# facebookresearch/fast3r

Measured on AMD Instinct MI355X. Metric: views/sec (512^2, ViT-L) single forward pass at N=320, higher is better.
Workload: dtype fp16

## Files before the change

fast3r_amd/_lib.py:

```python
import ctypes
import os

import torch

F3R_F16, F3R_BF16 = 0, 1
F3R_A_PLAIN, F3R_A_CONV3X3 = 0, 1
F3R_EPI_GENERIC, F3R_EPI_QKV, F3R_EPI_CONVT = 0, 1, 2
F3R_ACT_NONE, F3R_ACT_GELU, F3R_ACT_RELU = 0, 1, 2
F3R_SPLIT_NONE, F3R_SPLIT_W2, F3R_SPLIT_X3, F3R_SPLIT_W2F8, F3R_SPLIT_X3F8 = 0, 1, 2, 3, 4
F3R_MAX_SEG = 8
F3R_REAL_F32, F3R_REAL_F64 = 0, 1
F3R_LOSS_DIS, F3R_LOSS_LOG1P = 0, 1
SCENE_TILE = 4096
COLLECT_TILE = 1024
F3R_SKY_CLASSIFY, F3R_SKY_MORPH, F3R_SKY_LABEL = 1, 2, 4
F3R_SKY_EMPTY, F3R_SKY_NO_TOP, F3R_SKY_TOP = 0, 1, 2
SKY_PIX_TILE, SKY_WORD_TILE = 16, 256
MESH_TILE = 1024
F3R_INDEX_I32, F3R_INDEX_I64 = 0, 1
CLOUD_TILE, CLOUD_SORT_TILE, CLOUD_FPS_TILE, CLOUD_FPS_ONE_MAX = 1024, 2048, 1024, 8192
RENDER_CENTER_PARTS = 1024
RASTER_SMALL_PIXELS = 64
F3R_FPS_AUTO, F3R_FPS_ONE, F3R_FPS_TILED = 0, 1, 2
MAPS_TILE = 1024
F3R_MAPS_LUT, F3R_MAPS_RGB = 0, 1
GTVIEW_CAM_WORDS = 25
F3R_GTVIEW_POSE, F3R_GTVIEW_FINITE_MASK = 1, 2
DEPTH_TILE, DEPTH_ROW_WORDS, DEPTH_OUT_WORDS, DEPTH_MAX_THRESHOLDS = 1024, 8, 16, 4
F3R_DEPTH_ALIGN_NONE, F3R_DEPTH_ALIGN_MEDIAN = 0, 1
MATCH_TILE = 2048
F3R_CLEAN_WORLD, F3R_CLEAN_CAMERA = 0, 1
F3R_GALIGN_L1, F3R_GALIGN_L2 = 0, 1

_c_i64, _c_i32, _c_f32, _c_vp = ctypes.c_int64, ctypes.c_int32, ctypes.c_float, ctypes.c_void_p


class GemmArgs(ctypes.Structure):
    _fields_ = [
        ("A", _c_vp), ("W", _c_vp), ("bias", _c_vp),
        ("M", _c_i64), ("N", _c_i32), ("K", _c_i32), ("Kpad", _c_i32), ("lda", _c_i64),
        ("a_mode", _c_i32), ("a_relu", _c_i32),
        ("conv_H", _c_i32), ("conv_W", _c_i32), ("conv_C", _c_i32), ("conv_stride", _c_i32),
        ("conv_OH", _c_i32), ("conv_OW", _c_i32),
        ("epi", _c_i32), ("act", _c_i32),
        ("rowadd", _c_vp), ("rowadd_div", _c_i64),
        ("res_f32", _c_vp), ("ldr_f32", _c_i64),
        ("res_lp", _c_vp), ("ldr_lp", _c_i64),
        ("res_lp2", _c_vp), ("ldr_lp2", _c_i64),
        ("out_f32", _c_vp), ("ldo_f32", _c_i64),
        ("out_lp", _c_vp), ("ldo_lp", _c_i64),
        ("q", _c_vp), ("k", _c_vp), ("vt", _c_vp), ("seq_len", _c_i64), ("ldvt", _c_i64),
        ("rope_cos", _c_vp), ("rope_sin", _c_vp), ("rope_w", _c_i32), ("q_scale", _c_f32),
        ("ct_s", _c_i32), ("ct_h", _c_i32), ("ct_w", _c_i32), ("ct_cout", _c_i32),
        ("dtype", _c_i32), ("rope_mode", _c_i32),
        ("split", _c_i32), ("kernel_sel", _c_i32), ("A_lo", _c_vp),
        ("out_lp_lo", _c_vp), ("res_lp_lo", _c_vp), ("res_lp2_lo", _c_vp), ("out_relu", _c_vp), ("out_relu_lo", _c_vp),
        ("qkv_dq", _c_i32), ("out_lp_f8", _c_i32),
        ("w_scale", _c_vp), ("W_aux", _c_vp),
        ("out_f8", _c_vp), ("out_relu_f8", _c_vp),
        ("fin_w", _c_vp), ("fin_b", _c_vp), ("fin_pts", _c_vp), ("fin_conf", _c_vp),
        ("fin_n_out", _c_i32), ("fin_depth_mode", _c_i32), ("fin_conf_mode", _c_i32), ("fin_vmin", _c_f32), ("fin_vmax", _c_f32), ("reserved0", _c_i32),
    ]


class AttnArgs(ctypes.Structure):
    _fields_ = [
        ("q", _c_vp), ("o", _c_vp),
        ("ldq", _c_i64), ("ldo", _c_i64),
        ("q_batch_stride", _c_i64), ("o_batch_stride", _c_i64),
        ("tq", _c_i64),
        ("batch", _c_i32), ("n_heads", _c_i32), ("n_seg", _c_i32), ("dtype", _c_i32),
        ("k_seg", _c_vp * F3R_MAX_SEG), ("vt_seg", _c_vp * F3R_MAX_SEG),
        ("seg_len", _c_i64 * F3R_MAX_SEG), ("ldvt", _c_i64 * F3R_MAX_SEG),
        ("ldk", _c_i64),
        ("k_batch_stride", _c_i64 * F3R_MAX_SEG), ("vt_batch_stride", _c_i64 * F3R_MAX_SEG),
        ("scale", _c_f32), ("q_prescaled", _c_i32),
        ("st_o", _c_vp), ("st_ml", _c_vp), ("state_in", _c_i32), ("state_out", _c_i32),
        ("kv_group", _c_i32), ("causal", _c_i32), ("q_pos0", _c_i64), ("seg_pos0", _c_i64 * F3R_MAX_SEG),
        ("kernel_sel", _c_i32), ("head_dim", _c_i32),
        ("dbg_counters", _c_vp),
        ("sched_counter", _c_vp),
        ("qk_planes", _c_i32), ("reserve_cus", _c_i32),
    ]


class AttnF32Args(ctypes.Structure):
    _fields_ = [
        ("q", _c_vp), ("k", _c_vp), ("v", _c_vp), ("ldq", _c_i64), ("ldkv", _c_i64),
        ("o_hi", _c_vp), ("o_lo", _c_vp), ("o_f32", _c_vp), ("ldo", _c_i64),
        ("n_seq", _c_i64), ("tq", _c_i64), ("tk", _c_i64), ("q_pos0", _c_i64), ("k_pos0", _c_i64),
        ("n_heads", _c_i32), ("kv_group", _c_i32), ("causal", _c_i32), ("dtype", _c_i32), ("head_dim", _c_i32), ("scale", _c_f32),
    ]


SYMBOLS = {
    "f3r_version": (ctypes.c_int, []),
    "f3r_last_error_string": (ctypes.c_char_p, []),
    "f3r_sizeof": (ctypes.c_size_t, [ctypes.c_int]),
    "f3r_wall_clock_khz": (ctypes.c_int, []),
    "f3r_patchify": (ctypes.c_int, [_c_vp, _c_vp, ctypes.c_int, ctypes.c_int, ctypes.c_int, ctypes.c_int, ctypes.c_int, ctypes.c_int, _c_vp]),
    "f3r_interp_bilinear": (ctypes.c_int, [_c_vp, _c_vp, _c_vp, _c_vp] + [ctypes.c_int] * 9 + [_c_vp]),
    "f3r_interp_bilinear_f8": (ctypes.c_int, [_c_vp, _c_vp, _c_vp, _c_vp, _c_vp] + [ctypes.c_int] * 9 + [_c_vp]),
    "f3r_layernorm": (ctypes.c_int, [_c_vp, _c_vp, _c_vp, _c_vp, _c_vp, _c_i64, ctypes.c_int, _c_f32, ctypes.c_int, ctypes.c_int, _c_vp]),
    "f3r_layernorm_f8": (ctypes.c_int, [_c_vp, _c_vp, _c_vp, _c_vp, _c_i64, _c_i64, ctypes.c_int, _c_f32, ctypes.c_int, _c_vp]),
    "f3r_gemm": (ctypes.c_int, [ctypes.POINTER(GemmArgs), _c_vp]),
    "f3r_attn_fwd": (ctypes.c_int, [ctypes.POINTER(AttnArgs), _c_vp]),
    "f3r_attn_kernel_name": (ctypes.c_char_p, [ctypes.POINTER(AttnArgs)]),
    "f3r_block_workspace_bytes": (ctypes.c_size_t, [_c_i64, ctypes.c_int, ctypes.c_int, ctypes.c_int, _c_i64, _c_i64, ctypes.POINTER(ctypes.c_size_t)]),
    "f3r_block_workspace_bytes_ex": (ctypes.c_size_t, [_c_i64, ctypes.c_int, ctypes.c_int, ctypes.c_int, _c_i64, _c_i64, ctypes.c_int, ctypes.POINTER(ctypes.c_size_t)]),
    "f3r_upsample2x": (ctypes.c_int, [_c_vp, _c_vp, _c_vp, _c_vp, ctypes.c_int, ctypes.c_int, ctypes.c_int, ctypes.c_int, ctypes.c_int, ctypes.c_int, ctypes.c_int, _c_vp]),
    "f3r_dpt_final": (ctypes.c_int, [_c_vp, _c_vp, _c_vp, _c_vp, ctypes.c_int, _c_vp, _c_vp, _c_i64, ctypes.c_int, ctypes.c_int, ctypes.c_int,
                                     _c_f32, _c_f32, ctypes.c_int, _c_vp]),
    "f3r_cast_f32_to_lp": (ctypes.c_int, [_c_vp, _c_vp, _c_vp, _c_i64, ctypes.c_int, _c_vp]),
    "f3r_align_workspace_bytes": (ctypes.c_size_t, [ctypes.c_int]),
    "f3r_align_local_to_global": (ctypes.c_int, [_c_vp, _c_vp, _c_vp, _c_vp, _c_vp, _c_vp, _c_vp, _c_vp, ctypes.c_size_t,
                                                 ctypes.c_int, _c_i64, _c_f32, _c_vp]),
    "f3r_focal_workspace_bytes": (ctypes.c_size_t, [ctypes.c_int, ctypes.c_int, ctypes.c_int]),
    "f3r_estimate_focal": (ctypes.c_int, [_c_vp, _c_vp, _c_vp, _c_vp, _c_vp, ctypes.c_size_t, ctypes.c_int, ctypes.c_int, ctypes.c_int,
                                          _c_f32, _c_f32, _c_f32, ctypes.c_int, _c_f32, _c_f32, _c_vp]),
    "f3r_nn_index_bytes": (ctypes.c_size_t, [_c_i64]),
    "f3r_nn_workspace_bytes": (ctypes.c_size_t, [_c_i64]),
    "f3r_nn_build": (ctypes.c_int, [_c_vp, _c_i64, _c_vp, ctypes.c_size_t, _c_vp, ctypes.c_size_t, _c_vp]),
    "f3r_nn_query": (ctypes.c_int, [_c_vp, _c_vp, _c_i64, _c_vp, _c_vp, _c_vp, ctypes.c_size_t, _c_vp]),
    "f3r_estimate_normals": (ctypes.c_int, [_c_vp, _c_vp, ctypes.c_int, _c_vp, _c_vp, _c_vp, _c_vp]),
    "f3r_recon_stats_workspace_bytes": (ctypes.c_size_t, [_c_i64]),
    "f3r_recon_stats": (ctypes.c_int, [_c_vp, _c_vp, _c_vp, _c_vp, _c_i64, _c_i64, ctypes.c_double, _c_vp, _c_vp, ctypes.c_size_t, _c_vp]),
    "f3r_recon_prepare_workspace_bytes": (ctypes.c_size_t, [ctypes.c_int, ctypes.c_int, _c_i64]),
    "f3r_recon_prepare": (ctypes.c_int, [_c_vp, _c_vp, _c_vp, _c_vp, _c_vp, ctypes.c_int, ctypes.c_int, _c_i64, _c_f32, _c_f32, _c_vp, _c_vp,
                                         _c_vp, _c_vp, _c_vp, ctypes.c_size_t, _c_vp]),
    "f3r_resample_u8": (ctypes.c_int, [_c_vp, _c_vp, ctypes.c_int, ctypes.c_int, ctypes.c_int, ctypes.c_int, _c_vp, _c_vp, ctypes.c_int, _c_vp]),
    "f3r_imgnorm_u8": (ctypes.c_int, [_c_vp, _c_vp, ctypes.c_int, ctypes.c_int, ctypes.c_int, ctypes.c_int, ctypes.c_int, ctypes.c_int, _c_vp]),
    "f3r_silu_mul": (ctypes.c_int, [_c_vp, _c_vp, _c_i64, ctypes.c_int, ctypes.c_int, _c_vp]),
    "f3r_rows_add_f32": (ctypes.c_int, [_c_vp, _c_vp, _c_i64, ctypes.c_int, _c_vp]),
    "f3r_rope2d_f32": (ctypes.c_int, [_c_vp, _c_i64, _c_i64, ctypes.c_int, _c_i64, ctypes.c_int, _c_vp, _c_vp, _c_vp]),
    "f3r_attn_f32": (ctypes.c_int, [_c_vp, _c_vp, _c_vp, _c_i64, _c_vp, _c_vp, _c_vp, _c_i64, _c_i64, _c_i64, ctypes.c_int, _c_f32, ctypes.c_int, ctypes.c_int, _c_vp]),
    "f3r_rope_f32": (ctypes.c_int, [_c_vp, _c_i64, _c_i64, ctypes.c_int, _c_i64, ctypes.c_int, ctypes.c_int, _c_vp, _c_vp, _c_vp]),
    "f3r_silu_mul_f32": (ctypes.c_int, [_c_vp, _c_vp, _c_vp, _c_i64, ctypes.c_int, ctypes.c_int, _c_vp]),
    "f3r_attn_f32_ex": (ctypes.c_int, [ctypes.POINTER(AttnF32Args), _c_vp]),
    "f3r_attn_f32_mfma_workspace": (ctypes.c_int64, [ctypes.POINTER(AttnF32Args)]),
    "f3r_attn_f32_mfma": (ctypes.c_int, [ctypes.POINTER(AttnF32Args), _c_vp, ctypes.c_int64, _c_vp]),
    "f3r_qkv_planes": (ctypes.c_int, [_c_vp, _c_i64, _c_i64, _c_i64, ctypes.c_int, ctypes.c_int, _c_f32, _c_vp, _c_vp, _c_vp, _c_i64, ctypes.c_int, ctypes.c_int, _c_vp]),
    "f3r_attn_state_finish": (ctypes.c_int, [_c_vp, _c_vp, _c_i64, ctypes.c_int, ctypes.c_int, _c_vp, _c_vp, _c_vp, _c_i64, ctypes.c_int, _c_vp]),
    "f3r_estimate_poses": (ctypes.c_int, [_c_vp, _c_vp, _c_vp, _c_vp, _c_vp, _c_vp, ctypes.c_int, ctypes.c_int, ctypes.c_int, _c_f32, _c_f32,
                                          _c_f32, ctypes.c_int, ctypes.c_int, _c_vp]),
    "f3r_pose_pair_metrics": (ctypes.c_int, [_c_vp, _c_vp, ctypes.c_int, ctypes.c_int, ctypes.c_int, ctypes.POINTER(ctypes.c_double), ctypes.c_int,
                                             ctypes.POINTER(ctypes.c_double), ctypes.c_int, ctypes.c_int, ctypes.c_double, _c_vp, _c_vp, _c_vp, _c_vp]),
    "f3r_pose_error_stats": (ctypes.c_int, [_c_vp, _c_vp, _c_i64, ctypes.c_int, ctypes.POINTER(ctypes.c_double), ctypes.c_int,
                                            ctypes.POINTER(ctypes.c_double), ctypes.c_int, ctypes.c_int, ctypes.c_double, _c_vp, _c_vp]),
    "f3r_mv_conf_loss_workspace_bytes": (ctypes.c_size_t, [ctypes.c_int, ctypes.c_int]),
    "f3r_mv_conf_loss": (ctypes.c_int, [_c_vp, _c_vp, _c_vp, ctypes.c_int, _c_vp, _c_vp, _c_vp, _c_vp, _c_vp, ctypes.c_int, ctypes.c_int, ctypes.c_int,
                                        ctypes.c_int, ctypes.c_int, ctypes.c_int, ctypes.c_int, ctypes.c_double, ctypes.c_double, _c_vp, ctypes.c_size_t,
                                        _c_vp, _c_vp]),
    "f3r_scene_sort_workspace_bytes": (ctypes.c_size_t, [_c_i64, _c_i64]),
    "f3r_scene_sort": (ctypes.c_int, [_c_vp, ctypes.c_int, _c_i64, _c_i64, _c_vp, _c_vp, ctypes.c_size_t, _c_vp, _c_vp, _c_vp, _c_vp, _c_vp, _c_vp,
                                      _c_vp, _c_vp]),
    "f3r_scene_extent_workspace_bytes": (ctypes.c_size_t, []),
    "f3r_scene_extent": (ctypes.c_int, [_c_vp, _c_i64, ctypes.POINTER(_c_i64), _c_vp, ctypes.c_size_t, _c_vp, _c_vp]),
    "f3r_scene_collect_count": (ctypes.c_int, [_c_vp, ctypes.c_int, _c_i64, _c_vp, _c_vp]),
    "f3r_scene_collect_write": (ctypes.c_int, [_c_vp, ctypes.c_int, _c_i64, _c_vp, _c_vp, _c_vp, _c_vp]),
    "f3r_ply_pack": (ctypes.c_int, [_c_vp, _c_vp, _c_i64, _c_vp, _c_vp]),
# ... 18 lines not shown
    "f3r_cloud_voxel_sums": (ctypes.c_int, [_c_vp, _c_vp, _c_i64, _c_i64, _c_vp, ctypes.c_size_t, _c_vp, _c_vp, _c_vp, _c_vp]),
    "f3r_cloud_fps_workspace_bytes": (ctypes.c_size_t, [_c_i64]),
    "f3r_cloud_fps": (ctypes.c_int, [_c_vp, _c_i64, _c_i64, _c_i64, ctypes.c_int, _c_vp, ctypes.c_size_t, _c_vp, _c_vp]),
    "f3r_cloud_mark": (ctypes.c_int, [_c_vp, _c_i64, _c_i64, _c_vp, _c_vp]),
    "f3r_cloud_gather": (ctypes.c_int, [_c_vp, _c_vp, _c_vp, ctypes.c_int, _c_i64, _c_i64, _c_vp, _c_vp, _c_vp]),
    "f3r_render_clear": (ctypes.c_int, [_c_vp, ctypes.c_int, ctypes.c_int, _c_vp]),
    "f3r_render_splat": (ctypes.c_int, [_c_vp, _c_i64, _c_i64, _c_i64, ctypes.POINTER(ctypes.c_double), ctypes.c_double, ctypes.c_int, ctypes.c_int,
                                        _c_vp, _c_vp]),
    "f3r_render_resolve": (ctypes.c_int, [_c_vp, _c_vp, _c_i64, ctypes.c_int, ctypes.c_int, ctypes.c_uint32, _c_vp, _c_vp, _c_vp]),
    "f3r_render_center": (ctypes.c_int, [_c_vp, _c_i64, _c_vp, _c_vp, _c_vp]),
    "f3r_raster_workspace_bytes": (ctypes.c_size_t, [_c_i64]),
    "f3r_raster_triangles": (ctypes.c_int, [_c_vp, _c_i64, _c_vp, ctypes.c_int, _c_i64, _c_i64, _c_i64, _c_i64, ctypes.POINTER(ctypes.c_double),
                                            ctypes.c_int, ctypes.c_int, _c_vp, _c_vp, ctypes.c_size_t, _c_i64, _c_vp]),
    "f3r_maps_colorize": (ctypes.c_int, [_c_vp, ctypes.POINTER(_c_i64), ctypes.c_int, _c_i64, ctypes.c_int, _c_vp, _c_vp, _c_vp, _c_vp]),
    "f3r_gtview_workspace_bytes": (ctypes.c_size_t, [ctypes.c_int, ctypes.c_int, ctypes.c_int]),
    "f3r_gtview_resample": (ctypes.c_int, [_c_vp] + [ctypes.c_int] * 5 + [_c_vp, _c_vp, ctypes.c_int, ctypes.c_int, _c_vp, _c_vp] + [ctypes.c_int] * 9
                            + [_c_vp, _c_vp, _c_vp, ctypes.c_size_t, _c_vp]),
    "f3r_gtview_unproject": (ctypes.c_int, [_c_vp, _c_vp] + [ctypes.c_int] * 5 + [_c_vp, _c_vp] + [ctypes.c_int] * 8 + [_c_vp, _c_vp, _c_vp, _c_vp, _c_vp]),
    "f3r_depth_workspace_bytes": (ctypes.c_size_t, [ctypes.c_int, _c_i64, _c_i64, ctypes.c_int, ctypes.c_int]),
    "f3r_depth_medians": (ctypes.c_int, [_c_vp, ctypes.POINTER(_c_i64), ctypes.c_int, _c_i64, ctypes.c_int, ctypes.c_int, _c_f32, _c_vp, _c_i64, _c_vp]),
    "f3r_depth_errors": (ctypes.c_int, [_c_vp, ctypes.POINTER(_c_i64), ctypes.c_int, _c_i64, ctypes.c_int, ctypes.c_int, ctypes.c_double,
                                        ctypes.c_double, ctypes.POINTER(ctypes.c_double), ctypes.c_int, _c_vp, ctypes.c_size_t, _c_vp, _c_i64, _c_vp]),
    "f3r_depth_sparsify": (ctypes.c_int, [_c_vp, ctypes.POINTER(_c_i64), ctypes.c_int, _c_i64, ctypes.c_int, ctypes.c_int, ctypes.c_double,
                                          ctypes.c_double, ctypes.c_int, _c_vp, ctypes.c_size_t, _c_vp, _c_vp, _c_vp, _c_vp, _c_i64, _c_vp]),
    "f3r_match_index_bytes": (ctypes.c_size_t, [ctypes.POINTER(_c_i64), ctypes.c_int]),
    "f3r_match_workspace_bytes": (ctypes.c_size_t, [_c_i64, ctypes.c_int]),
    "f3r_match_index": (ctypes.c_int, [_c_vp, _c_vp, ctypes.POINTER(_c_i64), ctypes.c_int, _c_vp, ctypes.c_size_t, _c_vp, ctypes.c_size_t, _c_vp]),
    "f3r_match_search": (ctypes.c_int, [_c_vp, ctypes.POINTER(_c_i64), ctypes.c_int, _c_vp, ctypes.POINTER(_c_i32), _c_vp, ctypes.POINTER(_c_i64),
                                        ctypes.c_int, _c_vp, _c_vp, _c_vp]),
    "f3r_match_count": (ctypes.c_int, [_c_vp, _c_vp, ctypes.POINTER(_c_i64), ctypes.c_int, _c_vp, ctypes.POINTER(_c_i32), _c_vp,
                                       ctypes.POINTER(_c_i64), ctypes.c_int, _c_vp, ctypes.POINTER(_c_i64), ctypes.c_int, _c_vp, _c_vp, _c_vp, _c_vp]),
    "f3r_match_write": (ctypes.c_int, [_c_vp, ctypes.POINTER(_c_i64), ctypes.c_int, _c_vp, ctypes.POINTER(_c_i32), _c_vp, ctypes.POINTER(_c_i64),
                                       ctypes.c_int, _c_vp, ctypes.POINTER(_c_i64), ctypes.c_int, _c_vp, _c_vp, _c_vp, _c_vp, _c_vp, _c_vp, _c_vp, _c_vp,
                                       _c_i64, _c_vp]),
    "f3r_clean_workspace_bytes": (ctypes.c_size_t, [ctypes.c_int]),
    "f3r_clean_confidence": (ctypes.c_int, [_c_vp, _c_vp, _c_vp, _c_vp, _c_vp, _c_vp, ctypes.POINTER(_c_i64), ctypes.c_int, _c_vp,
                                            ctypes.POINTER(_c_i32), _c_i64, ctypes.c_double, _c_f32, ctypes.c_int, _c_vp, _c_vp, _c_vp, _c_vp,
                                            ctypes.c_size_t, _c_vp]),
    "f3r_galign_workspace_bytes": (ctypes.c_size_t, [ctypes.c_int, ctypes.c_int]),
    "f3r_galign_loss_grad": (ctypes.c_int, [_c_vp] * 7 + [ctypes.POINTER(_c_i64), ctypes.c_int, _c_vp, ctypes.POINTER(_c_i32), ctypes.c_int, _c_vp,
                                            ctypes.POINTER(_c_i64), _c_vp, ctypes.POINTER(_c_i32), ctypes.c_int] + [_c_vp] * 8
                             + [ctypes.c_size_t, _c_vp]),
}

SYMBOL_SINCE = {name: 420 for name in SYMBOLS if name.startswith("f3r_cloud_")}
SYMBOL_SINCE_430 = {name: 430 for name in SYMBOLS if name.startswith("f3r_render_")}
SYMBOL_IF_PRESENT = frozenset(name for name in SYMBOLS if name.startswith("f3r_raster_"))
SYMBOL_IF_PRESENT_MAPS = frozenset(name for name in SYMBOLS if name.startswith("f3r_maps_"))
SYMBOL_IF_PRESENT_VIEWS = frozenset(name for name in SYMBOLS if name.startswith("f3r_gtview_"))
SYMBOL_IF_PRESENT_DEPTH = frozenset(name for name in SYMBOLS if name.startswith("f3r_depth_"))
SYMBOL_IF_PRESENT_MATCH = frozenset(name for name in SYMBOLS if name.startswith("f3r_match_"))
SYMBOL_IF_PRESENT_CLEAN = frozenset(name for name in SYMBOLS if name.startswith("f3r_clean_"))
SYMBOL_IF_PRESENT_GALIGN = frozenset(name for name in SYMBOLS if name.startswith("f3r_galign_"))


def symbol_since(name: str) -> int:
    return SYMBOL_SINCE.get(name, SYMBOL_SINCE_430.get(name, 0))


def if_present(name: str) -> bool:
    return (name in SYMBOL_IF_PRESENT or name in SYMBOL_IF_PRESENT_MAPS or name in SYMBOL_IF_PRESENT_VIEWS or name in SYMBOL_IF_PRESENT_DEPTH
            or name in SYMBOL_IF_PRESENT_MATCH or name in SYMBOL_IF_PRESENT_CLEAN or name in SYMBOL_IF_PRESENT_GALIGN)


LIB_PATH = os.path.join(os.path.dirname(os.path.abspath(__file__)), "lib", "libf3r_hip.so")
if os.environ.get("F3R_LAB_LIB"):
    LIB_PATH = os.environ["F3R_LAB_LIB"]
_lib = None


class F3RError(RuntimeError):
    pass


ABI_VERSION = 410


def lib():
    global _lib
    if _lib is None:
        if not os.path.exists(LIB_PATH):
            raise F3RError(f"{LIB_PATH} not found: build it with `python -c 'import __graft_entry__ as g; g.build()'` "
                           "(fast3r_amd has no CPU / torch fallback)")
        l = ctypes.CDLL(LIB_PATH)

        def bind(name):
            fn = getattr(l, name)
            fn.restype, fn.argtypes = SYMBOLS[name]

        bind("f3r_version")
        if l.f3r_version() < ABI_VERSION:
            raise F3RError(f"{LIB_PATH} is version {l.f3r_version()}, this host code needs >= {ABI_VERSION}: rebuild it (fast3r_amd/csrc/build.sh)")
        for name in SYMBOLS:
            if if_present(name) and not hasattr(l, name):
                continue
            if symbol_since(name) <= l.f3r_version():
                bind(name)
        if l.f3r_sizeof(0) != ctypes.sizeof(GemmArgs) or l.f3r_sizeof(1) != ctypes.sizeof(AttnArgs) or l.f3r_sizeof(2) != ctypes.sizeof(AttnF32Args):
            raise F3RError("fast3r_amd/_lib.py struct layout does not match include/f3r.h "
                           f"(gemm {l.f3r_sizeof(0)} vs {ctypes.sizeof(GemmArgs)}, attn {l.f3r_sizeof(1)} vs {ctypes.sizeof(AttnArgs)}, "
                           f"attn_f32 {l.f3r_sizeof(2)} vs {ctypes.sizeof(AttnF32Args)}): rebuild the library (fast3r_amd/csrc/build.sh)")
        _lib = l
    return _lib


def library_version() -> int:
    return lib().f3r_version()


def entry(name: str):
    l = lib()
    have, need = library_version(), symbol_since(name)
    if have < need:
        raise F3RError(f"{LIB_PATH} is version {have}, {name} needs >= {need}: rebuild it (fast3r_amd/csrc/build.sh)")
# ... 44 lines not shown
```

fast3r_amd/csrc/asm/attn_gen.py:

```python
#!/usr/bin/env python3
import sys
import os

sys.path.insert(0, os.path.dirname(os.path.abspath(__file__)))
from isa import Program, Ins, Label, LabelRef, Lit, Neg, V, A, S, VCC, M0, EXEC, Reg

ARG_Q, ARG_O = 0, 8
ARG_LDQ = 16
ARG_NTILES = 32
ARG_QBS = 40
ARG_KVSHIFT = 56
ARG_STO = 64
ARG_KBS = 80
ARG_STLD = 96
ARG_TQ = 104
ARG_SEG = 112
SEG_BYTES = 24
ARG_DBG = ARG_SEG + 8 * SEG_BYTES
ARG_SCHED = ARG_DBG + 8
ARG_SIZE = ARG_SCHED + 32
FLAG_STATE_IN, FLAG_STATE_OUT = 1, 2

N_SLOTS = 4

s_q, s_k, s_vt, s_o = S(8, 2), S(10, 2), S(12, 2), S(14, 2)
s_ldq, s_ldk, s_ldvt, s_ldo = S(16), S(17), S(18), S(19)
s_nt, s_nseg = S(20), S(21)
s_wid, s_t, s_dma_u, s_seg_left = S(22), S(23), S(24), S(25)
s_kstep = S(26, 2)
s_m0base, s_seg, s_hopret, s_flags = S(28), S(29), S(30), S(31)
s_sto = S(32, 2)
s_lomask = S(34, 2)
s_ret, s_floor, s_ntm1 = S(36), S(37), S(38)
SEG0 = 52
s_stml = S(100, 2)


def seg_rec(i):
    return S(SEG0 + 6 * i, 2), S(SEG0 + 6 * i + 2, 2), S(SEG0 + 6 * i + 4)



s_delta = S(39)
s_shift = S(5)
s_tq = S(6)
s_rebase = S(7)
s_t0cyc, s_t0rt = S(SEG0 + 5), S(SEG0 + 11)

LANE = 0
s_mixrel = S(51)


class AttnGen:
    def __init__(self, dtype="f16", rowsum="pkadd", big_gap=None, k8_gap=2, name=None, ablate=(), cvt="rne", dma_aux="", dma_start=8, dma_step=None, pf=None, nslot=4,
                 fold="dot", head_dim=64, qk_planes=1, corr="f16", qk3_queues=True, k_hoist=True, qpw=None, tiles_per_barrier=1):
        assert dtype in ("f16", "bf16")
        assert head_dim in (64, 80, 128), "head widths with a generated kernel"
        assert qk_planes in (1, 2) and (qk_planes == 1 or (head_dim == 64 and dtype == "f16")) and corr in ("f16", "f8") and (corr == "f16" or qk_planes == 2)
        self.qk_planes, self.corr = qk_planes, corr
        self.qk3_queues = bool(qk3_queues)
        self.k_hoist = k_hoist
        self.dtype = dtype
        if rowsum == "pkadd" and dtype != "f16":
            rowsum = "add"
        self.rowsum = rowsum
        D = self.D = head_dim
        DK = self.DK = D * qk_planes
        assert qpw in (None, 2, 4) and (qpw is None or (head_dim == 64 and qk_planes == 1))
        self.QPW = QPW = qpw or (4 if (D == 64 and qk_planes == 1) else 2)
        self.WG_Q = 4 * QPW * 32
        self.NK = DK // 16
        self.QK_STEPS = ([(i, i) for i in range(self.NK)] if qk_planes == 1 else
                         [(i, i) for i in range(4)] + [(4 + i, i) for i in range(4)] + [(i, 4 + i) for i in range(4)])
        if corr == "f8":
            self.QK_STEPS = [(i, i) for i in range(4)] + [(6, 4, "f8", "unit", "lo"), (4, 6, "f8", "lo", "unit")]
        self.NQK = len(self.QK_STEPS)
        self.NDB = (D + 31) // 32
        self.DLAST = (D - 32 * (self.NDB - 1)) // 8
        self.KGROUPS = {64: [(0, 64)], 128: [(0, 64), (8192, 64)], 80: [(0, 64), (8192, 16)]}[DK]
        self.V_OFF = {64: 8192, 128: 16384, 80: 10240}[DK]
        self.SLOT = {64: 16384, 128: 32768, 80: 24576}[D] if qk_planes == 1 else 24576
        self.NP = 2 * (DK // 64) + (1 if D == 80 else 0) + 2 * (D // 64)
        if dma_step is None:
            dma_step = 6 if (D == 64 and qk_planes == 1 and self.QPW == 4) else 2
        self.dma_aux, self.dma_start, self.dma_step = dma_aux, dma_start, dma_step
        if pf is None:
            pf = 3 if corr == "f8" else 2
            if tiles_per_barrier > 1:
                pf = tiles_per_barrier + 1
        G = self.G = int(tiles_per_barrier)
        assert nslot in (4, 8) and G >= 1 and G + 1 <= pf and pf + G <= nslot, "LDS ring: G + 1 <= pf (read after write) and pf + G <= nslot (write after read)"
        assert D == 64 or nslot == 4
        assert G == 1 or (D == 64 and qk_planes == 1 and self.QPW == 4)
        self.pf, self.nslot = pf, nslot
        self.fold = fold
        self.LDS_X = nslot * self.SLOT
        self.lds_bytes = nslot * self.SLOT + 16
        v = 12
        self.S_BASE = v; v += 2 * QPW * 16
        self.P_BASE = v; v += QPW * 8
        self.NEGM = v; v += QPW * 16
        self.E_BASE = v; v += 4
        self.PSUM = v; v += QPW
        self.LRUN = v; v += QPW
        self.KCUR = v; v += 4
        self.VCUR = v; v += 4
        self.KREM = None
        if D == 80:
            self.KREM = v; v += 1
        self.SC_UNIT = self.SC_LO = None
        if corr == "f8":
            self.SC_UNIT = v; self.SC_LO = v + 1; v += 2
        a = 0
        self.O_BASE = a; a += QPW * self.NDB * 16
        self.Q_BASE = a; a += QPW * self.NK * 4
        self.KF_BASE = a; a += self.NK * 4
        self.VF_BASE = a; a += 2 * self.NDB * 4
        if a + self.NP <= 256:
            self.DOFF, self.doff_in_agpr = a, True
            a += self.NP
        else:
            self.DOFF, self.doff_in_agpr = v, False
            v += self.NP
        assert v <= 256 and a <= 256
        self.agpr_count = (a + 7) // 8 * 8
        pcs = []
        for goff, cols in self.KGROUPS:
            if cols == 64:
                pcs += [("A", "k", goff), ("A", "k", goff + 1024)]
        if D == 80:
            pcs.append(("A", "mix", None))
        for blk in range(D // 64):
            pcs += [("B", "vt", self.V_OFF + 8192 * blk), ("B", "vt", self.V_OFF + 8192 * blk + 1024)]
        assert len(pcs) == self.NP
        self.pieces = [(st, base, i, rel) for i, (st, base, rel) in enumerate(pcs)]
        if big_gap is None:
            big_gap = 4 if rowsum == "pkadd" else 5
        self.big_gap, self.k8_gap = (tuple(big_gap) if isinstance(big_gap, (tuple, list)) else (int(big_gap),)), k8_gap
        self.ablate = set(ablate)
        self.name = name or (f"f3r_attn_asm_q256_{dtype}" if (D == 64 and qk_planes == 1 and self.QPW == 2) else f"f3r_attn_asm_qk3f8_{dtype}" if corr == "f8" else f"f3r_attn_asm_qk3_{dtype}" if qk_planes == 2 else f"f3r_attn_asm_{dtype}" if D == 64 else f"f3r_attn_asm_d{D}_{dtype}")
        if name is None and G > 1:
            self.name += "_grp"
        self.p = Program(self.name)
        if dtype == "f16":
            self.MFMA, self.MFMA8 = "v_mfma_f32_32x32x16_f16", "v_mfma_f32_32x32x8_f16"
            self.CVT, self.DOT, self.ONE2 = "v_cvt_pk_f16_f32", "v_dot2c_f32_f16", 0x3C003C00
            if cvt == "rtz":
                self.CVT = "v_cvt_pkrtz_f16_f32"
        else:
            self.MFMA, self.MFMA8 = "v_mfma_f32_32x32x16_bf16", "v_mfma_f32_32x32x8bf16_1k"
            self.CVT, self.DOT, self.ONE2 = "v_cvt_pk_bf16_f32", "v_dot2c_f32_bf16", 0x3F803F80

    def Sv(self, e, qb, r=None):
        base = self.S_BASE + e * self.QPW * 16 + qb * 16
        return V(base, 16) if r is None else V(base + r)

    def Pv(self, qb, ks, j=None):
        base = self.P_BASE + qb * 8 + ks * 4
        return V(base, 4) if j is None else V(base + j)

    def Nv(self, qb, r=None):
        base = self.NEGM + qb * 16
        return V(base, 16) if r is None else V(base + r)

    def Oa(self, qb, db, r=None):
        base = self.O_BASE + (qb * self.NDB + db) * 16
        return A(base, 16) if r is None else A(base + r)

    def Qa(self, qb, ds):
        return A(self.Q_BASE + (qb * self.NK + ds) * 4, 4)

    def KFa(self, ds):
        return A(self.KF_BASE + ds * 4, 4)

    def VFa(self, j):
        return A(self.VF_BASE + j * 4, 4)

    def rq_range(self, db):
        return range(4 if db < self.NDB - 1 else self.DLAST)

    def mul_const(self, dst, src, c, comment=""):
        if c & (c - 1) == 0:
            self.e("s_lshl_b32", dst, src, c.bit_length() - 1, comment=comment)
        else:
            self.e("s_mul_i32", dst, src, Lit(c), comment=comment)

    def k_read(self, ds, half):
        grp, rem = divmod(ds, 4)
        goff, cols = self.KGROUPS[grp]
        if cols == 64:
            return self.I("ds_read_b128", self.KFa(ds), V(self.KCUR + rem), offset=goff + 4096 * half)
        return self.I("ds_read_b128", self.KFa(ds), V(self.KREM), offset=1024 * half)

    def I(self, op, *args, comment="", **mods):
        return Ins(op, tuple(args), dict(mods), comment)
# ... 621 lines not shown

    def epilogue(self):
        e = self.e
        e("s_waitcnt", "vmcnt(0)", comment="re-issued tail tiles of the LDS-DMA stream")
        e("s_nop", 15)
        e("s_nop", 15)
        e("s_load_dwordx2", S(40, 2), S(0, 2), Lit(ARG_DBG))
        e("s_waitcnt", "lgkmcnt(0)")
        e("s_cmp_eq_u64", S(40, 2), 0)
        e("s_cbranch_scc1", self.L("NO_DBG"))
        e("s_memtime", S(42, 2))
        e("s_memrealtime", S(44, 2))
        e("v_mov_b32", V(8), 0)
        e("v_mov_b32", V(9), s_rebase)
        e("v_mov_b32", V(10), 1)
        e("v_mov_b32", V(12), s_nt)
        e("v_mov_b32", V(13), 0)
        e("s_waitcnt", "lgkmcnt(0)")
        e("s_sub_u32", S(42), S(42), s_t0cyc, comment="cycles of this wave (a wave lives < 2^32 cycles: the low words suffice)")
        e("s_sub_u32", S(44), S(44), s_t0rt)
        e("v_mov_b32", V(14), S(42))
        e("v_mov_b32", V(15), 0)
        e("v_mov_b32", V(16), S(44))
        e("v_mov_b32", V(17), 0)
        e("s_mov_b64", EXEC, 1, comment="lane 0")
        e("global_atomic_add", V(8), V(9), S(40, 2))
        e("global_atomic_add", V(8), V(10), S(40, 2), offset=4)
        e("global_atomic_add_x2", V(8), V(12, 2), S(40, 2), offset=8)
        e("global_atomic_add_x2", V(8), V(14, 2), S(40, 2), offset=16)
        e("global_atomic_add_x2", V(8), V(16, 2), S(40, 2), offset=24)
        e("s_getreg_b32", S(46), "hwreg(HW_REG_XCC_ID, 0, 4)")
        e("s_and_b32", S(46), S(46), 7)
        e("s_mul_i32", S(46), S(46), 24)
        e("s_add_u32", S(48), S(40), S(46))
        e("s_addc_u32", S(49), S(41), 0)
        e("v_mov_b32", V(18), 1)
        e("v_mov_b32", V(19), 0)
        e("global_atomic_add_x2", V(8), V(14, 2), S(48, 2), offset=32)
        e("global_atomic_add_x2", V(8), V(16, 2), S(48, 2), offset=40)
        e("global_atomic_add_x2", V(8), V(18, 2), S(48, 2), offset=48)
        e("s_mov_b64", EXEC, -1)
        self.lab("NO_DBG")
        e("s_and_b32", S(40), s_flags, FLAG_STATE_OUT)
        e("s_cmp_lg_u32", S(40), 0)
        e("s_cbranch_scc1", self.L("STATE_OUT"))
        e("v_and_b32", V(2), 31, V(LANE))
        e("v_lshrrev_b32", V(3), 5, V(LANE))
        e("v_mul_lo_u32", V(4), V(2), s_ldo)
        e("v_lshlrev_b32", V(5), 3, V(3))
        e("v_add_u32", V(4), V(4), V(5), comment="lq * ldo + g * 8")
        e("v_xor_b32", V(7), 32, V(LANE))
        e("v_lshlrev_b32", V(7), 2, V(7), comment="(lane ^ 32) * 4")
        e("s_lshl_b32", S(47), s_ldo, 5)
        k = 0
        for qb in range(self.QPW):
            if qb:
                e("s_mov_b64", EXEC, -1)
                e("v_add_u32", V(4), S(47), V(4))
            e("ds_bpermute_b32", V(5), V(7), V(self.LRUN + qb))
            e("s_waitcnt", "lgkmcnt(0)")
            e("v_add_f32", V(5), V(5), V(self.LRUN + qb))
            e("v_rcp_f32", V(6), V(5))
            self.own_rows_mask(qb)
            for db in range(self.NDB):
                for rq in self.rq_range(db):
                    t = 16 + 6 * (k % 4)
                    k += 1
                    if k > 4 and (k - 1) % 4 == 0:
                        e("s_waitcnt", "vmcnt(0)")
                    for i in range(4):
                        e("v_accvgpr_read_b32", V(t + i), self.Oa(qb, db, rq * 4 + i))
                    for i in range(4):
                        e("v_mul_f32", V(t + i), V(t + i), V(6))
                    e(self.CVT, V(t + 4), V(t), V(t + 1))
                    e(self.CVT, V(t + 5), V(t + 2), V(t + 3))
                    e("global_store_dwordx2", V(4), V(t + 4, 2), s_o, offset=db * 64 + rq * 16)
        self.item_done()
        self.lab("STATE_OUT")
        self.state_rows_offsets()
        k = 0
        for qb in range(self.QPW):
            if qb:
                e("s_mov_b64", EXEC, -1, comment="(v_cmp writes 0 for inactive lanes: the mask of block qb must not inherit block qb-1's)")
            self.own_rows_mask(qb)
            for db in range(self.NDB):
                for rq in self.rq_range(db):
                    t = 32 + 4 * (k % 8)
                    k += 1
                    if k > 8 and (k - 1) % 8 == 0:
                        e("s_waitcnt", "vmcnt(0)")
                    for i in range(4):
                        e("v_accvgpr_read_b32", V(t + i), self.Oa(qb, db, rq * 4 + i))
                    e("global_store_dwordx4", V(16 + qb), V(t, 4), s_sto, offset=db * 128 + rq * 32)
                    e("s_nop", 1)
            e("v_xor_b32", V(28 + qb), Lit(0x80000000), self.Nv(qb, 0), comment="m = -NEGM")
            e("global_store_dword", V(20 + qb), V(28 + qb), s_stml)
            e("global_store_dword", V(24 + qb), V(self.LRUN + qb), s_stml, offset=4)
        self.item_done()

    def item_done(self):
        e = self.e
        e("s_mov_b64", EXEC, -1)
        e("s_load_dwordx2", S(40, 2), S(0, 2), Lit(ARG_SCHED))
        e("s_waitcnt", "lgkmcnt(0)")
        e("s_cmp_eq_u64", S(40, 2), 0)
        e("s_cbranch_scc0", self.L("FETCH"))
        e("s_endpgm")

    def fetch_block(self):
        e = self.e
        self.lab("FETCH")
        e("s_waitcnt", "vmcnt(0)", comment="this item's stores have read their registers")
        e("s_load_dwordx2", S(40, 2), S(0, 2), Lit(ARG_SCHED))
        e("s_load_dwordx4", S(44, 4), S(0, 2), Lit(ARG_SCHED + 8), comment="n_work, nx, nxy, magic(nx)")
        e("s_load_dwordx2", S(48, 2), S(0, 2), Lit(ARG_SCHED + 24), comment="magic(nxy), grid")
        e("s_waitcnt", "lgkmcnt(0)")
        e("s_barrier")
        e("s_cmp_eq_u32", s_wid, 0)
        e("s_cbranch_scc0", self.L("F_WAIT"))
        e("v_mov_b32", V(8), 0)
        e("v_mov_b32", V(9), 1)
        e("v_mov_b32", V(11), Lit(self.LDS_X))
        e("s_mov_b64", EXEC, 1, comment="lane 0")
        e("global_atomic_add", V(10), V(8), V(9), S(40, 2), text="sc0")
        e("s_waitcnt", "vmcnt(0)")
        e("ds_write_b32", V(11), V(10))
        e("s_waitcnt", "lgkmcnt(0)")
        e("s_mov_b64", EXEC, -1)
        self.lab("F_WAIT")
# ... 194 lines not shown
    .vgpr_count:     {256 + self.agpr_count}
    .vgpr_spill_count: 0
    .wavefront_size: 64
"""


AttnGen2 = AttnGen


def module_text(gens):
    out = ['\t.amdgcn_target "amdgcn-amd-amdhsa--gfx950"\n\t.amdhsa_code_object_version 6\n']
    for g in gens:
        out.append(g.text())
    out.append("\t.amdgpu_metadata\n---\namdhsa.kernels:\n")
    for g in gens:
        out.append(g.metadata())
    out.append("amdhsa.target:   amdgcn-amd-amdhsa--gfx950\namdhsa.version:\n  - 1\n  - 2\n...\n\n\t.end_amdgpu_metadata\n")
    return "".join(out)


HEAD_DIMS = (64, 80, 128)


GROUPED_RING = dict(tiles_per_barrier=2, pf=4, nslot=8)


def product_generators(ring=None, **kw):
    gens = []
    q3 = kw.pop("qk3_queues", True)
    kh = kw.pop("k_hoist", True)
    for hd in HEAD_DIMS:
        for dt in ("f16", "bf16"):
            g = AttnGen(dt, head_dim=hd, **(dict(kw, name=f"f3r_attn_asm_{dt}", **ring) if (ring and hd == 64) else kw))
            g.build()
            gens.append(g)
    kw3 = dict(kw)
    if kw3.get("dma_step") == 6:
        kw3["dma_step"] = None
    for dt in ("f16", "bf16"):
        g = AttnGen(dt, head_dim=64, qpw=2, **kw3)
        g.build()
        gens.append(g)
    for corr in ("f16", "f8"):
        g = AttnGen("f16", head_dim=64, qk_planes=2, corr=corr, qk3_queues=q3, k_hoist=kh, **kw3)
        g.build()
        gens.append(g)
    for dt in ("f16", "bf16"):
        g = AttnGen(dt, head_dim=64, **dict(kw, name=f"f3r_attn_asm_{dt}_grp", **(ring or GROUPED_RING)))
        g.build()
        gens.append(g)
    return gens


def main():
    import argparse
    ap = argparse.ArgumentParser()
    ap.add_argument("out")
    ap.add_argument("--rowsum", default="pkadd")
    ap.add_argument("--big-gap", default=None, help="fillers per MFMA gap: an int, or a comma list cycled over the gaps of a stage, e.g. 4,5")
    ap.add_argument("--k8-gap", type=int, default=2)
    ap.add_argument("--ablate", default="", help="comma list: nosoftmax,nodma,nobarrier,nolds,norare (timing only, wrong results)")
    ap.add_argument("--cvt", default="rne")
    ap.add_argument("--dma-aux", default="")
    ap.add_argument("--dma-start", type=int, default=8)
    ap.add_argument("--dma-step", type=int, default=6)
    ap.add_argument("--fold", default="dot")
    ap.add_argument("--layout", type=int, default=2, help="(accepted for old scripts; there is one layout)")
    ap.add_argument("--pf", type=int, default=None, help="tiles the LDS-DMA runs ahead (with --tiles-per-barrier / --nslot 8: of the 512-query head_dim-64 kernels only)")
    ap.add_argument("--nslot", type=int, default=4, help="LDS ring slots; 8: the 512-query head_dim-64 kernels only (the other slots do not fit eight times)")
    ap.add_argument("--tiles-per-barrier", type=int, default=None,
                    help="G: one s_barrier per G key tiles in every 512-query head_dim-64 kernel of the module, the _grp symbols included (1 with --nslot 4: all of them the plain form)")
    ap.add_argument("--qk3-queues", type=int, default=1, help="three-product kernels: 0 = in-order filler placement (measurement)")
    ap.add_argument("--k-hoist", type=int, default=1, help="fp8-correction kernel: 0 = K fragments requested in the stage that multiplies them (measurement)")
    a = ap.parse_args()
    bg = None if a.big_gap is None else (tuple(int(x) for x in a.big_gap.split(",")) if "," in a.big_gap else int(a.big_gap))
    ring = None
    if a.tiles_per_barrier is not None or a.nslot == 8:
        ring = dict(tiles_per_barrier=a.tiles_per_barrier or 1, pf=a.pf, nslot=a.nslot)
        a.pf, a.nslot = None, 4
    gens = product_generators(ring=ring, rowsum=a.rowsum, big_gap=bg, k8_gap=a.k8_gap, ablate=[x for x in a.ablate.split(",") if x], cvt=a.cvt,
                              dma_aux=a.dma_aux, dma_start=a.dma_start, dma_step=a.dma_step, pf=a.pf, nslot=a.nslot, fold=a.fold, qk3_queues=bool(a.qk3_queues), k_hoist=bool(a.k_hoist))
    for g in gens:
        problems = g.p.check_hazards() if not a.ablate else []
        if problems:
            sys.stderr.write("\n".join(problems[:40]) + f"\n{len(problems)} hazard(s) in {g.name}\n")
            sys.exit(1)
    with open(a.out, "w") as f:
        f.write(module_text(gens))


if __name__ == "__main__":
    main()
```

fast3r_amd/csrc/asm/gemm_gen.py:

```python
#!/usr/bin/env python3
import os
import struct
import sys

sys.path.insert(0, os.path.dirname(os.path.abspath(__file__)))
from isa import Program, Ins, Label, LabelRef, Lit, Neg, V, A, S, VCC, M0, EXEC

ARG_A, ARG_W, ARG_BIAS, ARG_RES, ARG_OUT = 0, 8, 16, 24, 32
ARG_LD = 40
ARG_NK = 56
ARG_MAP = 64
ARG_SEG = 96
ARG_SIZE = 128
ARG_F8 = 128
ARG_SIZE_F8 = 144
ARG_ROPE = 144
ARG_SIZE_LP = 176
FLAG_BIAS_ON_M = 1
FLAG_SKEW = 2
MIN_NK = 4
ACT_NONE, ACT_GELU, ACT_RELU, ACT_SCALE = 0, 1, 2, 3
ACT_ROPE = 4

SLOT = 32768
# ... 16 lines not shown
s_gc = [S(64 + i) for i in range(8)]
s_argOut, s_pw_base, s_pa_nbase, s_pw_nbase = S(72, 2), S(74, 2), S(76, 2), S(78, 2)
s_has_next, s_tile, s_tnext = S(80), S(81), S(82)
s_kw = S(83)
s_segstride, s_tps, s_tpsm, s_scale, s_flags, s_nk1w = S(84, 2), S(86), S(87), S(88), S(89), S(90)
s_scale_tile = S(91)
s_wsc, s_argWsc = S(92, 2), S(94, 2)
s_nk8 = S(61)
s_out8off, s_out8 = S(3), S(12, 2)

LANE = 0
FA_BASE, FW_BASE = 16, 48
AADDR, WADDR = 80, 92
OFFA, OFFW = 104, 112
VOFFO, VOFFR = 120, 124
BIASF, ONESF = 128, 144
GCV = 148
EPI = 152
EPX, EPT = 32, 64
VBIAS, VBOFF = 12, 11
SCW, VUNIT, AADDR8, WADDR8 = 224, 228, 232, 244
A8_BASE = {(0, 0): 16, (0, 1): 24, (0, 2): 48, (0, 3): 56, (1, 0): 32, (1, 1): 40, (1, 2): 64, (1, 3): 72}
W8_BASE = {(0, 0): 152, (0, 1): 160, (1, 0): 168, (1, 1): 176}


def FA(buf, j):
    return V(FA_BASE + buf * 16 + j * 4, 4)


def FW(buf, ib):
    return V(FW_BASE + buf * 16 + ib * 4, 4)


def ACC(ib, j, r=None, n=None):
    base = (ib * 4 + j) * 16
    if r is None:
        return A(base, 16)
    return A(base + r, n or 1)


def f32bits(x):
    return struct.unpack("<I", struct.pack("<f", x))[0]


def A8(b, j):
    return V(A8_BASE[(b, j)], 8)


def W8(p, x):
    return V(W8_BASE[(p, x)], 8)


class GemmGen:
    def __init__(self, dtype="f16", role="f32", name=None, ablate=(), f8=False):
        assert dtype in ("f16", "bf16") and role in ("f32", "lp")
        assert not (f8 and dtype != "f16"), "the fp8 low plane corrects fp16 planes (the split modes are an fp16 design)"
        self.dtype, self.role, self.f8 = dtype, role, f8
        self.perm = role == "lp"
        self.esize = 4 if role == "f32" else 2
        self.ablate = set(ablate)
        self.name = name or f"f3r_gemm_asm_{role}{'8' if f8 else ''}_{dtype}"
        self.arg_size = ARG_SIZE_LP if role == "lp" else (ARG_SIZE_F8 if f8 else ARG_SIZE)
        self.MFMA8 = "v_mfma_scale_f32_32x32x64_f8f6f4"
        self.lds_bytes = LDS_BYTES
        self.p = Program(self.name)
        self.MFMA = "v_mfma_f32_32x32x16_f16" if dtype == "f16" else "v_mfma_f32_32x32x16_bf16"
        self.CVT = "v_cvt_pk_f16_f32" if dtype == "f16" else "v_cvt_pk_bf16_f32"

    def I(self, op, *args, comment="", **mods):
        return Ins(op, tuple(args), dict(mods), comment)

    def e(self, op, *args, comment="", **mods):
        return self.p.emit(op, *args, comment=comment, **mods)

    def L(self, name):
        return LabelRef(f".L{self.name}_{name}")

    def lab(self, name):
        self.p.label(f".L{self.name}_{name}")

    def emit_all(self, lst):
        for ins in lst:
            self.p.items.append(ins)

    def mul64(self, dst, base, a, b, tmp):
        e = self.e
        e("s_mul_i32", tmp[0], a, b)
        e("s_mul_hi_u32", tmp[1], a, b)
        e("s_add_u32", dst.sub(0), base.sub(0), tmp[0])
        e("s_addc_u32", dst.sub(1), base.sub(1), tmp[1])

    def tile_map(self, tile):
        e = self.e
        e("s_and_b32", T[0], tile, 7, comment="xcd")
        e("s_lshr_b32", T[1], tile, 3, comment="idx")
        e("s_add_u32", T[2], s_xq, 1)
        e("s_mul_i32", T[3], T[0], T[2], comment="xcd * (q + 1)")
        e("s_mul_i32", T[4], s_xr, T[2], comment="r * (q + 1)")
        e("s_sub_u32", T[5], T[0], s_xr)
        e("s_mul_i32", T[5], T[5], s_xq)
        e("s_add_u32", T[4], T[4], T[5])
        e("s_cmp_lt_u32", T[0], s_xr)
        e("s_cselect_b32", T[3], T[3], T[4])
        e("s_add_u32", T[3], T[3], T[1], comment="position in the XCD-contiguous order")
        e("s_mul_hi_u32", T[4], T[3], s_pgm, comment="group = pos / (gm * n_tiles_n)")
        e("s_cmp_eq_u32", s_pg, 1, comment="(a divisor of one has no 32-bit magic number)")
        e("s_cselect_b32", T[4], T[3], T[4])
        e("s_mul_i32", T[5], T[4], s_pg)
        e("s_sub_u32", T[5], T[3], T[5], comment="position inside the group")
        e("s_lshr_b32", T[6], T[5], s_gsh, comment="tn")
        e("s_lshl_b32", T[7], 1, s_gsh)
        e("s_sub_u32", T[7], T[7], 1)
        e("s_and_b32", T[7], T[5], T[7])
        e("s_lshl_b32", T[4], T[4], s_gsh)
        e("s_add_u32", T[7], T[7], T[4], comment="tm")
        e("s_lshl_b32", T[8], T[7], 8, comment="m0")
        e("s_lshl_b32", T[9], T[6], 8, comment="n0")

    def stream_bases(self, dst_a, dst_w):
        self.mul64(dst_a, s_argA, T[8], s_lda, (T[0], T[1]))
        self.mul64(dst_w, s_argW, T[9], s_ldw, (T[0], T[1]))

    def bias_ptr(self):
        e = self.e
        e("s_lshl_b32", T[3], s_wn, 7)
        e("s_add_u32", T[3], T[3], T[9], comment="first output column of this wave")
        e("s_lshl_b32", T[2], s_wm, 7)
        e("s_add_u32", T[2], T[2], T[8], comment="first output row of this wave")
        e("s_and_b32", T[4], s_flags, FLAG_BIAS_ON_M)
        e("s_cmp_eq_u32", T[4], 0)
        e("s_cselect_b32", T[3], T[3], T[2])
        e("s_lshl_b32", T[4], T[3], 2)
        e("s_add_u32", s_bias.sub(0), s_argBias.sub(0), T[4])
        e("s_addc_u32", s_bias.sub(1), s_argBias.sub(1), 0)

    def wsc_ptr(self):
        e = self.e
        e("s_lshl_b32", T[3], s_wn, 7)
        e("s_add_u32", T[3], T[3], T[9], comment="first output column of this wave")
        e("s_lshl_b32", T[4], T[3], 2)
        e("s_add_u32", s_wsc.sub(0), s_argWsc.sub(0), T[4])
        e("s_addc_u32", s_wsc.sub(1), s_argWsc.sub(1), 0)

    def wsc_loads(self):
        e = self.e
        for ib in range(4):
            e("global_load_dword", V(SCW + ib), V(VBOFF), s_wsc, offset=128 * ib)

    def out_ptrs(self):
        e = self.e
        e("s_lshr_b32", T[5], T[9], 8, comment="tn")
        e("s_mul_hi_u32", T[6], T[5], s_tpsm)
        e("s_cmp_eq_u32", s_tps, 1)
        e("s_cselect_b32", T[6], T[5], T[6], comment="segment")
        e("s_mul_i32", T[7], T[6], s_tps)
        e("s_sub_u32", T[7], T[5], T[7])
        e("s_lshl_b32", T[7], T[7], 8, comment="first column of the tile inside its segment")
        e("s_cmp_eq_u32", T[6], 0)
        e("s_cselect_b32", s_scale_tile, s_scale, 1.0)
        e("s_lshl_b32", T[2], s_wm, 7)
        e("s_add_u32", T[2], T[2], T[8], comment="first token row of this wave")
        e("s_lshl_b32", T[3], s_wn, 7)
        e("s_add_u32", T[3], T[3], T[7], comment="first output column of this wave")
        self.mul64(s_out, s_argOut, T[2], s_ldo, (T[0], T[1]))
        e("s_lshl_b32", T[4], T[3], 2 if self.esize == 4 else 1)
        e("s_add_u32", s_out.sub(0), s_out.sub(0), T[4])
        e("s_addc_u32", s_out.sub(1), s_out.sub(1), 0)
        e("s_mul_i32", T[0], T[6], s_segstride.sub(0))
        e("s_mul_hi_u32", T[1], T[6], s_segstride.sub(0))
        e("s_mul_i32", T[4], T[6], s_segstride.sub(1))
        e("s_add_u32", T[1], T[1], T[4])
        e("s_add_u32", s_out.sub(0), s_out.sub(0), T[0])
        e("s_addc_u32", s_out.sub(1), s_out.sub(1), T[1])
        if self.role == "f32":
            self.mul64(s_res, s_argRes, T[2], s_ldr, (T[0], T[1]))
            e("s_lshl_b32", T[4], T[3], 2)
            e("s_add_u32", s_res.sub(0), s_res.sub(0), T[4])
            e("s_addc_u32", s_res.sub(1), s_res.sub(1), 0)
        elif self.f8:
            e("s_sub_u32", s_out8.sub(0), s_out.sub(0), T[3])
            e("s_subb_u32", s_out8.sub(1), s_out.sub(1), 0)
            e("s_add_u32", s_out8.sub(0), s_out8.sub(0), s_out8off)
            e("s_addc_u32", s_out8.sub(1), s_out8.sub(1), 0)

    def next_tile_bases(self):
        e = self.e
        e("s_add_u32", s_tnext, s_tile, s_grid)
        e("s_cmp_lt_u32", s_tnext, s_nwg)
        e("s_cselect_b32", s_has_next, 1, 0)
        e("s_cselect_b32", T[10], s_tnext, s_tile, comment="(no next tile: any valid tile, never used)")
        self.tile_map(T[10])
        self.stream_bases(s_pa_nbase, s_pw_nbase)
# ... 46 lines not shown
            e("s_cbranch_scc1", self.L(f"WR_{c}"))
            e("s_mov_b64", s_pw_base, s_pw_nbase)
            e("s_mov_b32", s_tw, 0)
            e("s_mov_b32", s_kw, 0)
            e("s_mov_b32", s_kwoff, 0)
            e("s_branch", self.L(f"WR_{c}"))

    def reads(self, slot_a, slot_w, ks):
        buf = ks & 1
        I = self.I

        def rw(ib):
            return I("ds_read_b128", FW(buf, ib), V(WADDR + (slot_w // 2) * 4 + ks), offset=(slot_w % 2) * SLOT + ib * 4096)

        def ra(j):
            return I("ds_read_b128", FA(buf, j), V(AADDR + (slot_a // 2) * 4 + ks), offset=(slot_a % 2) * SLOT + j * 4096)
        out = [rw(0), ra(0), ra(1), ra(2), ra(3), rw(1), rw(2), rw(3)]
        return [] if "nolds" in self.ablate else out

    def mfmas(self, ks):
        buf = ks & 1
        return [self.I(self.MFMA, ACC(ib, j), FW(buf, ib), FA(buf, j), ACC(ib, j)) for ib in range(4) for j in range(4)]

    def kstep(self, ks, fill):
        out = []
        for i, m in enumerate(self.mfmas(ks)):
            out.append(m)
            out += fill.get(i, [])
        return out

    def r8(self, dst, addr_base, slot, ks, block):
        a = addr_base + (slot // 2) * 4 + 2 * ks
        off = (slot % 2) * SLOT + block * 4096
        return [self.I("ds_read_b128", dst.sub(0, 4), V(a), offset=off), self.I("ds_read_b128", dst.sub(4, 4), V(a + 1), offset=off)]

    def reads8_first(self, slot_a, slot_w):
        out = self.r8(W8(0, 0), WADDR8, slot_w, 0, 0)
        for j in range(4):
            out += self.r8(A8(0, j), AADDR8, slot_a, 0, j)
        return out + self.r8(W8(0, 1), WADDR8, slot_w, 0, 1)

    def reads8_tail(self, slot_a, slot_w, q):
        nq = q + 1
        out = []
        for x in range(2):
            out += self.r8(W8(nq % 2, x), WADDR8, slot_w, nq // 2, 2 * (nq % 2) + x)
        if q < 2:
            for j in (2 * q, 2 * q + 1):
                out += self.r8(A8(1, j), AADDR8, slot_a, 1, j)
        return [] if "nolds" in self.ablate else out

    def mfmas8(self, q):
        ks, pair = q // 2, q % 2
        return [self.I(self.MFMA8, ACC(2 * pair + x, j), W8(q % 2, x), A8(ks % 2, j), ACC(2 * pair + x, j), V(SCW + 2 * pair + x), V(VUNIT), text="op_sel_hi:[0,0,0]")
                for x in range(2) for j in range(4)]

    def phase8(self, q, fill):
        out = []
        for i, m in enumerate(self.mfmas8(q)):
            out.append(m)
            out += fill.get(i, [])
        return out

    @staticmethod
    def spread(fill, items, gaps):
        for k, it in enumerate(items):
            fill.setdefault(gaps[k % len(gaps)], []).append(it)

    def bias_loads(self):
        e = self.e
        for ib in range(4):
            e("global_load_dword", V(VBIAS + ib), V(VBOFF), s_bias, offset=128 * ib)

    def bias_frags(self):
        e = self.e
        for ib in range(4):
            b = V(VBIAS + ib)
            if self.dtype == "f16":
                e("v_cvt_f16_f32", V(1), b)
                e("v_and_b32", V(1), Lit(0xFFFF), V(1), comment="hi")
                e("v_cvt_f32_f16", V(2), V(1))
                e("v_sub_f32", V(2), b, V(2), comment="b - hi (exact)")
                e("v_cvt_f16_f32", V(3), V(2))
                e("v_and_b32", V(3), Lit(0xFFFF), V(3), comment="lo")
                e("v_cvt_f32_f16", V(4), V(3))
                e("v_sub_f32", V(4), V(2), V(4))
                e("v_cvt_f16_f32", V(5), V(4))
                e("v_and_b32", V(5), Lit(0xFFFF), V(5), comment="lo2")
                e("v_lshlrev_b32", V(3), 16, V(3))
                e("v_or_b32", V(1), V(1), V(3), comment="(hi, lo)")
            else:
                e("v_and_b32", V(1), Lit(0xFFFF0000), b, comment="hi")
                e("v_sub_f32", V(2), b, V(1))
                e("v_and_b32", V(3), Lit(0xFFFF0000), V(2), comment="lo")
                e("v_sub_f32", V(4), V(2), V(3))
                e("v_lshrrev_b32", V(5), 16, V(4), comment="lo2")
                e("v_lshrrev_b32", V(1), 16, V(1))
                e("v_or_b32", V(1), V(1), V(3), comment="(hi, lo)")
            e("v_mov_b32", V(6), 0)
            e("v_cndmask_b32", V(BIASF + ib * 4), V(6), V(1), s_lomask)
            e("v_cndmask_b32", V(BIASF + ib * 4 + 1), V(6), V(5), s_lomask)

    def bias_mfmas(self):
        e = self.e
        self.k_bm = getattr(self, "k_bm", 0) + 1
        e("s_and_b32", T[0], s_flags, FLAG_BIAS_ON_M)
# ... 675 lines not shown


def pack_args(a, w, bias, res, out, lda_b, ldw_b, ldr_b, ldo_b, nk, nk1, ntm, ntn, act=ACT_NONE, grid=None, seg_stride=0, tps=None, scale=1.0, flags=0,
              nk1_w=None, wscale=None, nk8=0, out8_off=0, rope=None):
    assert nk >= MIN_NK
    n_wg = ntm * ntn
    grid = min(n_wg, 256) if grid is None else grid
    gm_shift = 3
    while ntm % (1 << gm_shift):
        gm_shift -= 1
    pg = (1 << gm_shift) * ntn
    magic = -(-(1 << 32) // pg) if pg > 1 else 0
    tps = ntn if tps is None else tps
    tmagic = -(-(1 << 32) // tps) if tps > 1 else 0
    b = struct.pack("<QQQQQIIIIII", a, w, bias, res, out, lda_b, ldw_b, ldr_b, ldo_b, nk, nk1)
    b += struct.pack("<IIIIIIII", n_wg // 8, n_wg % 8, pg, magic, gm_shift, act, grid, n_wg)
    b += struct.pack("<qIIfIII", seg_stride, tps, tmagic, scale, flags, nk if nk1_w is None else nk1_w, 0)
    assert len(b) == ARG_SIZE
    if wscale is not None or rope is not None:
        b += struct.pack("<QII", wscale or 0, nk8, out8_off)
        assert len(b) == ARG_SIZE_F8
    if rope is not None:
        cos, sin, seq_len, rope_w = rope
        mg = lambda d: -(-(1 << 32) // d) if d > 1 else 0
        b += struct.pack("<QQIIII", cos, sin, seq_len, mg(seq_len), rope_w, mg(rope_w))
        assert len(b) == ARG_SIZE_LP
    return b, grid


def tile_of(wg, ntm, ntn):
    n_wg = ntm * ntn
    gm_shift = 3
    while ntm % (1 << gm_shift):
        gm_shift -= 1
    pg = (1 << gm_shift) * ntn
    q, r = n_wg // 8, n_wg % 8
    xcd, idx = wg & 7, wg >> 3
    pos = (xcd * (q + 1) if xcd < r else r * (q + 1) + (xcd - r) * q) + idx
    grp, rem = pos // pg, pos % pg
    return (grp << gm_shift) + (rem & ((1 << gm_shift) - 1)), rem >> gm_shift


def product_generators(**kw):
    gens = []
    for role in ("f32", "lp"):
        for dt in ("f16", "bf16"):
            g = GemmGen(dt, role, **kw)
            g.build()
            gens.append(g)
    for role in ("f32", "lp"):
        g = GemmGen("f16", role, f8=True, **kw)
        g.build()
        gens.append(g)
    return gens


def module_text(gens):
    out = ['\t.amdgcn_target "amdgcn-amd-amdhsa--gfx950"\n\t.amdhsa_code_object_version 6\n']
    for g in gens:
        out.append(g.text())
    out.append("\t.amdgpu_metadata\n---\namdhsa.kernels:\n")
    for g in gens:
        out.append(g.metadata())
    out.append("amdhsa.target:   amdgcn-amd-amdhsa--gfx950\namdhsa.version:\n  - 1\n  - 2\n...\n\n\t.end_amdgpu_metadata\n")
    return "".join(out)


def main():
    import argparse
    ap = argparse.ArgumentParser()
    ap.add_argument("out")
    ap.add_argument("--ablate", default="", help="comma list: nodma,nolds,nobarrier (timing only, wrong results)")
    a = ap.parse_args()
    gens = product_generators(ablate=[x for x in a.ablate.split(",") if x])
    for g in gens:
        problems = g.p.check_hazards() if not a.ablate else []
        if problems:
            sys.stderr.write("\n".join(problems[:40]) + f"\n{len(problems)} hazard(s) in {g.name}\n")
            sys.exit(1)
    with open(a.out, "w") as f:
        f.write(module_text(gens))


if __name__ == "__main__":
    main()
```

fast3r_amd/csrc/f3r_attn.hip:

```cpp
#include "f3r_common.h"
#include "f3r_dispatch.h"

namespace {

constexpr int AT_KB = 64;
constexpr int AT_TILE = 64 * 64;
constexpr int AT_NW = 4;
constexpr int AT_QPW = 2;
constexpr int AT_QB = AT_NW * AT_QPW * 32;
constexpr int AT_DPW = 8 / AT_NW;
constexpr float AT_REBASE_SUM = 64.f;

__device__ __forceinline__ int aswz(int row, int chunk) { return row * 64 + ((chunk ^ ((row >> 1) & 7)) << 3); }

template <class T, bool BATCHED, bool CAUSAL>
__global__ __launch_bounds__(AT_NW * 64, 2) void attn_kernel(const f3r_attn_args p) {
  constexpr int QPW = AT_QPW, DPW = AT_DPW;
  __shared__ __attribute__((aligned(16))) uint16_t lds[2 * 2 * AT_TILE];
  const int tid = threadIdx.x;
  const int lane = tid & 63;
  const int wid = __builtin_amdgcn_readfirstlane(tid >> 6);
  const int lq = lane & 31;
  const int g = lane >> 5;

// ... 310 lines not shown
  F3R_REQUIRE(a.q_batch_stride % 8 == 0 && a.o_batch_stride % 4 == 0, "f3r_attn_fwd: batch strides alignment");
  int64_t total = 0;
  for (int s = 0; s < a.n_seg; ++s) {
    F3R_REQUIRE(a.seg_len[s] >= 0, "f3r_attn_fwd: negative segment length");
    if (a.seg_len[s] == 0) continue;
    F3R_REQUIRE(a.k_seg[s] && a.vt_seg[s], "f3r_attn_fwd: null K/V^T segment %d", s);
    F3R_REQUIRE((((uintptr_t)a.k_seg[s]) & 15) == 0 && (((uintptr_t)a.vt_seg[s]) & 15) == 0, "f3r_attn_fwd: K/V^T alignment");
    F3R_REQUIRE(a.ldvt[s] % 64 == 0 && a.ldvt[s] >= a.seg_len[s], "f3r_attn_fwd: ldvt[%d]=%lld must be a multiple of 64 covering the segment (zero padded)", s,
                (long long)a.ldvt[s]);
    F3R_REQUIRE(a.k_batch_stride[s] % 8 == 0 && a.vt_batch_stride[s] % 8 == 0, "f3r_attn_fwd: K/V^T batch stride alignment");
    F3R_REQUIRE((int64_t)64 * a.ldk * 2 < (1ll << 32) && (int64_t)64 * a.ldvt[s] * 2 < (1ll << 32), "f3r_attn_fwd: ldk / ldvt too large for 32-bit tile offsets");
    total += a.seg_len[s];
  }
  F3R_REQUIRE(total > 0, "f3r_attn_fwd: no keys");
  if (a.causal && !a.state_in) {
    int first = 0;
    while (a.seg_len[first] == 0) ++first;
    F3R_REQUIRE(a.seg_pos0[first] <= a.q_pos0,
                "f3r_attn_fwd: causal launch without carried state whose first key (seg_pos0[%d] = %lld) lies after its first query (q_pos0 = %lld): "
                "the first key of a fresh launch must be visible to every query row (start from the shard that holds the queries, resume over the others)",
                first, (long long)a.seg_pos0[first], (long long)a.q_pos0);
  }
  F3R_REQUIRE(a.kv_group >= 0 && (a.kv_group <= 1 || a.n_heads % a.kv_group == 0), "f3r_attn_fwd: kv_group %d does not divide n_heads %d", a.kv_group, a.n_heads);
  const int kv_heads = a.kv_group > 1 ? a.n_heads / a.kv_group : a.n_heads;
  F3R_REQUIRE(a.ldk >= kv_heads * hd * qkp, "f3r_attn_fwd: ldk < kv heads * head_dim");
  F3R_REQUIRE(!(a.state_in || a.state_out) || (a.st_o && a.st_ml && al16(a.st_o) && al16(a.st_ml)), "f3r_attn_fwd: state buffers null/misaligned");
  F3R_REQUIRE(a.kernel_sel >= ATTN_SEL_AUTO && a.kernel_sel <= ATTN_SEL_ASM, "f3r_attn_fwd: kernel_sel %d", a.kernel_sel);
  return F3R_OK;
}

}

int f3r_attn_plan(const f3r_attn_args& a, AttnPlan* plan) {
  *plan = AttnPlan{};
  const int hd = attn_head_dim(a);
  const bool planes = a.qk_planes >= 2;
  const char* why = "kernel_sel 1";
  auto unsupported = [&why](const char* fmt) { f3r_set_error(fmt, why); return F3R_ERR_UNSUPPORTED; };
  const int64_t min_keys = (planes || a.kernel_sel == ATTN_SEL_ASM || hd != 64) ? 0 : F3R_ATTN_ASM_MIN_KEYS;
  if (a.kernel_sel != ATTN_SEL_HIP && f3r_attn_asm_plan(a, min_keys, plan, &why)) return F3R_OK;
  if (planes) return unsupported("f3r_attn_fwd: qk_planes 2 / 3 but the launch is not eligible for the hand-scheduled three-product kernel: %s");
  if (a.kernel_sel == ATTN_SEL_ASM) return unsupported("f3r_attn_fwd: kernel_sel 2 (hand-scheduled kernel) but the launch is not eligible: %s");
  plan->family = hd != 64 ? ATTN_GENERIC : (a.causal ? ATTN_HIP_CAUSAL : (a.batch > 1 ? ATTN_HIP_BATCHED : ATTN_HIP));
  return F3R_OK;
}

extern "C" const char* f3r_attn_kernel_name(const f3r_attn_args* args) {
  static const char* const hip[] = {"attn_kernel<causal> (f3r_attn.hip)", "attn_kernel<batched> (f3r_attn.hip)", "attn_kernel (f3r_attn.hip)", "attn_generic_kernel (f3r_attn_generic.hip)"};
  AttnPlan p;
  if (!args || f3r_attn_plan(*args, &p) != F3R_OK) return "";
  return p.family == ATTN_ASM ? f3r_attn_asm_name(*args, p) : hip[p.family];
}

extern "C" int f3r_attn_fwd(const f3r_attn_args* args, f3r_stream_t stream) {
  F3R_REQUIRE(args != nullptr, "f3r_attn_fwd: null args");
  const f3r_attn_args& a = *args;
  AttnPlan p;
  int rc = attn_validate(a);
  if (rc != F3R_OK || a.tq == 0) return rc;
  rc = f3r_attn_plan(a, &p);
  if (rc != F3R_OK) return rc;
  hipStream_t s = (hipStream_t)stream;
  if (p.family == ATTN_ASM) return f3r_attn_asm_launch(a, p, s);
  if (p.family == ATTN_GENERIC) return f3r_attn_generic_launch(a, s);
  return a.dtype == F3R_F16 ? attn_launch<F16>(a, p.family, s) : attn_launch<BF16>(a, p.family, s);
}
```

fast3r_amd/csrc/f3r_attn_asm.hip:

```cpp
#include <cstddef>
#include <cstdlib>
#include <cstring>

#include "f3r_common.h"
#include "f3r_dispatch.h"

extern "C" const unsigned char f3r_attn_asm_hsaco[];
extern "C" const unsigned int f3r_attn_asm_hsaco_len;

namespace {

struct f3r_attn_asm_seg {
  const void* k;
  const void* vt;
  uint32_t tiles, pad;
};
struct f3r_attn_asm_args {
  const void* q;
  void* o;
  uint32_t ldq_b, ldk_b, ldvt_b, ldo_b;
  uint32_t n_tiles, n_seg;
  uint64_t q_bs, o_bs;
  uint32_t kv_shift, flags;
  float* st_o;
  float* st_ml;
  uint64_t k_bs, vt_bs;
  uint32_t st_o_ld_b, st_ml_ld_b;
  uint32_t tq, pad;
  f3r_attn_asm_seg seg[8];
  uint32_t* dbg;
  uint32_t* sched;
  uint32_t n_work, nx, nxy, nx_magic, nxy_magic, grid;
};
static_assert(sizeof(f3r_attn_asm_args) == 344 && offsetof(f3r_attn_asm_args, seg) == 112 && offsetof(f3r_attn_asm_args, dbg) == 304 &&
              offsetof(f3r_attn_asm_args, sched) == 312 && offsetof(f3r_attn_asm_args, n_work) == 320,
              "must match ARG_SIZE / ARG_SEG / ARG_DBG / ARG_SCHED of attn_gen.py");

constexpr int kNumHd = 3, kHd[kNumHd] = {64, 80, 128};
int hd_index(int hd) {
  for (int i = 0; i < kNumHd; ++i)
    if (kHd[i] == hd) return i;
  return -1;
}
AttnItem native_item(int hd, int planes) { return (hd == 64 && planes < 2) ? ATTN_ITEM_512 : ATTN_ITEM_256; }

F3rCodeObject<12> g_kernels = {f3r_attn_asm_hsaco,
                               {"f3r_attn_asm_f16", "f3r_attn_asm_bf16", "f3r_attn_asm_d80_f16", "f3r_attn_asm_d80_bf16", "f3r_attn_asm_d128_f16", "f3r_attn_asm_d128_bf16",
                                "f3r_attn_asm_qk3_f16", "f3r_attn_asm_qk3f8_f16", "f3r_attn_asm_q256_f16", "f3r_attn_asm_q256_bf16", "f3r_attn_asm_f16_grp",
                                "f3r_attn_asm_bf16_grp"}};

hipFunction_t get_fn(int dtype, int hi, int planes, AttnItem item, bool grouped = false) {
  if (dtype < 0 || dtype > 1 || hi < 0) return nullptr;
  const bool hd64 = kHd[hi] == 64;
  if (planes >= 2) return (hd64 && dtype == F3R_F16) ? g_kernels.get(4 + planes) : nullptr;
  if (item != native_item(kHd[hi], planes)) return hd64 ? g_kernels.get(8 + dtype) : nullptr;
  if (grouped) return hd64 ? g_kernels.get(10 + dtype) : nullptr;
  return g_kernels.get(2 * hi + dtype);
}

bool pow2(int x) { return x > 0 && (x & (x - 1)) == 0; }

bool q256_wins(int64_t tq, int64_t hb, int64_t cus) {
  const int64_t n512 = (tq + 511) / 512 * hb, n256 = (tq + 255) / 256 * hb;
  const double t512 = (double)((n512 + cus - 1) / cus), t256 = 0.64 * (double)((n256 + cus - 1) / cus);
  return t256 < 0.97 * t512;
}

int64_t tail_split_rows(int64_t tq, int64_t hb, int64_t cus) {
  const int64_t nqb = (tq + 511) / 512;
  if (nqb * hb <= cus) return 0;
  int64_t x = cus, y = hb;
  while (y) { const int64_t t = x % y; x = y; y = t; }
  const int64_t g = cus / x;
  const int64_t nqb_main = nqb / g * g;
  if (nqb_main == 0 || nqb_main == nqb) return 0;
  if (nqb_main * hb / cus > 8) return 0;
  const int64_t r = (nqb - nqb_main) * hb;
  if (2 * r > cus) return 0;
  return nqb_main * 512;
}

void plan_items(const f3r_attn_args& a, AttnPlan& p) {
  const int hd = kHd[p.hd_index];
  p.main.rows = a.tq;
  p.main.item = native_item(hd, p.planes);
  if (p.main.item != ATTN_ITEM_512 || get_fn(a.dtype, p.hd_index, p.planes, ATTN_ITEM_256) == nullptr) return;
  static const char* force = getenv("F3R_ATTN_Q256");
  static const char* split = getenv("F3R_ATTN_TAIL_SPLIT");
  if (force && (force[0] == '0' || force[0] == '1')) {
    if (force[0] == '1') p.main.item = ATTN_ITEM_256;
    return;
  }
  const int64_t cus = f3r_device_cus(), hb = (int64_t)a.n_heads * a.batch;
  const bool may_split = !(split && split[0] == '0') && !a.state_in && !a.state_out && a.reserve_cus <= 0;
  const int64_t rows = may_split ? tail_split_rows(a.tq, hb, cus) : 0;
  if (rows > 0) {
    const AttnItem item = q256_wins(a.tq - rows, hb, cus) ? ATTN_ITEM_256 : ATTN_ITEM_512;
    if (a.tq - rows >= attn_item_wave_rows(item)) {
      p.main.rows = rows;
      p.tail.rows = a.tq - rows;
      p.tail.item = item;
      return;
    }
  }
  if (q256_wins(a.tq, hb, cus)) p.main.item = ATTN_ITEM_256;
}
// ... 22 lines not shown
  int first = -1;
  int64_t keys = 0;
  for (int s = 0; s < a.n_seg; ++s) {
    if (a.seg_len[s] == 0) continue;
    if (a.seg_len[s] % 64 != 0) { *why = "a K/V segment is not a multiple of 64 keys"; return false; }
    if (first < 0) first = s;
    if (a.ldvt[s] != a.ldvt[first] || a.k_batch_stride[s] != a.k_batch_stride[first] || a.vt_batch_stride[s] != a.vt_batch_stride[first]) {
      *why = "K/V segments with different ldvt / batch strides";
      return false;
    }
    keys += a.seg_len[s];
  }
  if (first < 0) { *why = "no keys"; return false; }
  if (keys < min_keys) { *why = "fewer keys than F3R_ATTN_ASM_MIN_KEYS"; return false; }
  if (keys / 64 >= (1ll << 31)) { *why = "too many keys"; return false; }
  if (wrows * a.ldq * 2 >= (1ll << 32) || wrows * a.ldo * 2 >= (1ll << 32) || 64 * a.ldk * 2 >= (1ll << 32) || (int64_t)hd * a.ldvt[first] * 2 >= (1ll << 32) ||
      wrows * a.n_heads * hd * 4 >= (1ll << 32)) {
    *why = "row strides too large for 32-bit lane offsets";
    return false;
  }
  if (a.tq >= (1ll << 31) || a.n_heads >= 65536 || a.batch >= 65536) { *why = "grid too large"; return false; }
  if (get_fn(a.dtype, hi, qkp, native_item(hd, qkp)) == nullptr) { *why = "the embedded code object could not be loaded on this device"; return false; }
  plan->family = ATTN_ASM;
  plan->hd_index = hi;
  plan->planes = qkp;
  plan_launches(a, keys, *plan);
  return true;
}

const char* f3r_attn_asm_name(const f3r_attn_args& a, const AttnPlan& p) {
  const bool h = a.dtype == F3R_F16;
  if (p.planes == 2) return "f3r_attn_asm_qk3_f16 (hand-scheduled, three products per score block, csrc/asm/attn_gen.py)";
  if (p.planes == 3) return "f3r_attn_asm_qk3f8_f16 (hand-scheduled, three products per score block, the corrections on the fp8 MFMA, csrc/asm/attn_gen.py)";
  if (kHd[p.hd_index] == 80) return h ? "f3r_attn_asm_d80_f16 (hand-scheduled, csrc/asm/attn_gen.py)" : "f3r_attn_asm_d80_bf16 (hand-scheduled, csrc/asm/attn_gen.py)";
  if (kHd[p.hd_index] == 128) return h ? "f3r_attn_asm_d128_f16 (hand-scheduled, csrc/asm/attn_gen.py)" : "f3r_attn_asm_d128_bf16 (hand-scheduled, csrc/asm/attn_gen.py)";
  if (p.tail.rows > 0 && p.main.grouped)
    return h ? "f3r_attn_asm_f16_grp + f3r_attn_asm_q256_f16 for the last round (hand-scheduled, one barrier per group of key tiles, csrc/asm/attn_gen.py)"
             : "f3r_attn_asm_bf16_grp + f3r_attn_asm_q256_bf16 for the last round (hand-scheduled, one barrier per group of key tiles, csrc/asm/attn_gen.py)";
  if (p.tail.rows > 0)
    return h ? "f3r_attn_asm_f16 + f3r_attn_asm_q256_f16 for the last round (hand-scheduled, csrc/asm/attn_gen.py)"
             : "f3r_attn_asm_bf16 + f3r_attn_asm_q256_bf16 for the last round (hand-scheduled, csrc/asm/attn_gen.py)";
  if (p.main.item == ATTN_ITEM_256)
    return h ? "f3r_attn_asm_q256_f16 (hand-scheduled, 256-query work items, csrc/asm/attn_gen.py)" : "f3r_attn_asm_q256_bf16 (hand-scheduled, 256-query work items, csrc/asm/attn_gen.py)";
  if (p.main.grouped)
    return h ? "f3r_attn_asm_f16_grp (hand-scheduled, one barrier per group of key tiles, csrc/asm/attn_gen.py)"
             : "f3r_attn_asm_bf16_grp (hand-scheduled, one barrier per group of key tiles, csrc/asm/attn_gen.py)";
  return h ? "f3r_attn_asm_f16 (hand-scheduled, csrc/asm/attn_gen.py)" : "f3r_attn_asm_bf16 (hand-scheduled, csrc/asm/attn_gen.py)";
}

static int launch_one(const f3r_attn_args& a, const AttnPlan& p, int64_t row0, const AttnAsmLaunch& l, hipStream_t stream) {
  const int hd = kHd[p.hd_index];
  const int wave_rows = attn_item_wave_rows(l.item);
  F3R_REQUIRE(l.rows >= wave_rows, "f3r_attn_fwd: a hand-scheduled launch of %lld query rows, fewer than the %d of one wave", (long long)l.rows, wave_rows);
  hipFunction_t fn = get_fn(a.dtype, p.hd_index, p.planes, l.item, l.grouped);
  if (!fn) {
    f3r_set_error("f3r_attn_fwd: the embedded hand-scheduled kernel could not be loaded on this device");
    return F3R_ERR_LAUNCH;
  }
  f3r_attn_asm_args k;
  memset(&k, 0, sizeof(k));
  k.q = (const char*)a.q + row0 * a.ldq * 2;
  k.o = (char*)a.o + row0 * a.ldo * 2;
  k.ldq_b = (uint32_t)(a.ldq * 2);
  k.ldk_b = (uint32_t)(a.ldk * 2);
  k.ldo_b = (uint32_t)(a.ldo * 2);
  k.q_bs = (uint64_t)a.q_batch_stride * 2;
  k.o_bs = (uint64_t)a.o_batch_stride * 2;
  int sh = 0;
  for (int gsz = a.kv_group > 1 ? a.kv_group : 1; gsz > 1; gsz >>= 1) ++sh;
  k.kv_shift = (uint32_t)sh;
  k.flags = (a.state_in ? 1u : 0u) | (a.state_out ? 2u : 0u);
  k.st_o = a.st_o;
  k.st_ml = a.st_ml;
  k.st_o_ld_b = (uint32_t)a.n_heads * (uint32_t)hd * 4u;
  k.st_ml_ld_b = (uint32_t)a.n_heads * 16u;
  k.tq = (uint32_t)l.rows;
  k.dbg = a.dbg_counters;
  for (int s = 0; s < a.n_seg; ++s) {
    if (a.seg_len[s] == 0) continue;
    f3r_attn_asm_seg& g = k.seg[k.n_seg++];
    g.k = a.k_seg[s];
    g.vt = a.vt_seg[s];
    g.tiles = (uint32_t)(a.seg_len[s] / 64);
    k.n_tiles += g.tiles;
    k.ldvt_b = (uint32_t)(a.ldvt[s] * 2);
    k.k_bs = (uint64_t)a.k_batch_stride[s] * 2;
    k.vt_bs = (uint64_t)a.vt_batch_stride[s] * 2;
  }
  const int64_t wg_rows = 4 * wave_rows;
  const unsigned nx = (unsigned)((l.rows + wg_rows - 1) / wg_rows);
  unsigned gx = nx, gy = (unsigned)a.n_heads, gz = (unsigned)a.batch;
  const uint64_t n_work = (uint64_t)nx * gy * gz, nxy = (uint64_t)nx * gy;
  unsigned cus = (unsigned)f3r_device_cus();
  const unsigned reserve = a.reserve_cus > 0 ? (unsigned)a.reserve_cus : 0u;
  const bool reserving = a.sched_counter && reserve > 0 && reserve < cus && n_work > (uint64_t)(cus - reserve);
  if (reserving) cus -= reserve;
  if (a.sched_counter && (reserving || n_work >= 2ull * cus) && n_work * nxy < (1ull << 32)) {
    k.sched = a.sched_counter;
    k.n_work = (uint32_t)n_work;
    k.nx = nx;
    k.nxy = (uint32_t)nxy;
    k.nx_magic = nx > 1 ? (uint32_t)(((1ull << 32) + nx - 1) / nx) : 0;
    k.nxy_magic = nxy > 1 ? (uint32_t)(((1ull << 32) + nxy - 1) / nxy) : 0;
    k.grid = cus;
    gx = cus;
    gy = gz = 1;
    hipError_t me = hipMemsetAsync(a.sched_counter, 0, 2 * sizeof(uint32_t), stream);
    if (me != hipSuccess) {
      f3r_set_error("f3r_attn_fwd: clearing sched_counter failed: %s", hipGetErrorString(me));
      return F3R_ERR_LAUNCH;
    }
  }
  size_t size = sizeof(k);
  void* config[] = {HIP_LAUNCH_PARAM_BUFFER_POINTER, &k, HIP_LAUNCH_PARAM_BUFFER_SIZE, &size, HIP_LAUNCH_PARAM_END};
  hipError_t e = hipModuleLaunchKernel(fn, gx, gy, gz, 256, 1, 1, 0, stream, nullptr, config);
  if (e != hipSuccess) {
    f3r_set_error("f3r_attn_fwd: hipModuleLaunchKernel failed: %s", hipGetErrorString(e));
    return F3R_ERR_LAUNCH;
  }
  return f3r_check_launch("f3r_attn_fwd(asm)");
}

int f3r_attn_asm_launch(const f3r_attn_args& a, const AttnPlan& p, hipStream_t stream) {
  const int rc = launch_one(a, p, 0, p.main, stream);
  return (rc != F3R_OK || p.tail.rows == 0) ? rc : launch_one(a, p, p.main.rows, p.tail, stream);
}
```

fast3r_amd/csrc/f3r_dispatch.h:

```cpp
#pragma once
#include <atomic>
#include <map>
#include <mutex>

#include "f3r_common.h"

inline bool al16(const void* p) { return (((uintptr_t)p) & 15) == 0; }
inline bool al8(const void* p) { return (((uintptr_t)p) & 7) == 0; }

inline int f3r_device_cus() {
  static std::atomic<int> cache[64];
  int dev = 0, cu = 0;
  if (hipGetDevice(&dev) != hipSuccess) dev = 0;
  std::atomic<int>* slot = (dev >= 0 && dev < 64) ? &cache[dev] : nullptr;
  if (slot && (cu = slot->load(std::memory_order_relaxed)) != 0) return cu;
  if (hipDeviceGetAttribute(&cu, hipDeviceAttributeMultiprocessorCount, dev) != hipSuccess || cu < 8) cu = 256;
  if (slot) slot->store(cu, std::memory_order_relaxed);
  return cu;
}
inline int f3r_num_cus() { return f3r_device_cus() / 8 * 8; }

template <int N>
struct F3rCodeObject {
  const unsigned char* image;
// ... 54 lines not shown
int f3r_gemm256_max_conv_k_tiles();
int f3r_gemm256_launch(const f3r_gemm_args& a, hipStream_t stream, const GemmPlan& plan);
bool f3r_gemm_asm_eligible(const f3r_gemm_args& a, const char** why);
bool f3r_gemm_asm_f8_eligible(const f3r_gemm_args& a, const char** why);
bool f3r_gemm_asm_qkv_eligible(const f3r_gemm_args& a, const char** why);
bool f3r_gemm_asm_preferred(int64_t tiles);
int f3r_gemm_asm_launch(const f3r_gemm_args& a, hipStream_t stream, const GemmPlan& plan);

inline float tile_score(int64_t tiles, int slots, float eff) {
  if (tiles <= 0) return 0.f;
  const int64_t rounds = (tiles + slots - 1) / slots;
  return eff * (float)tiles / (float)(rounds * slots);
}
inline float score_256(const f3r_gemm_args& a, int nh) {
  return tile_score(((a.M + 255) / 256) * ((a.N + 128 * nh - 1) / (128 * nh)), 256, nh == 2 ? 1.0f : 0.82f);
}
inline float score_128(const f3r_gemm_args& a) { return tile_score(((a.M + 127) / 128) * ((a.N + 127) / 128), 512, 0.72f); }

inline int f3r_gemm256_halves(const f3r_gemm_args& a, int forced) {
  if (a.epi == F3R_EPI_QKV) return 2;
  if (a.N % 256 != 0 || forced == 1) return 1;
  if (forced == 2) return 2;
  return score_256(a, 1) > score_256(a, 2) ? 1 : 2;
}
inline bool f3r_gemm256_preferred(const f3r_gemm_args& a) { return score_256(a, f3r_gemm256_halves(a, 0)) >= score_128(a); }

enum {
  ATTN_SEL_AUTO = 0,
  ATTN_SEL_HIP = 1,
  ATTN_SEL_ASM = 2,
};
enum AttnFamily {
  ATTN_HIP_CAUSAL,
  ATTN_HIP_BATCHED,
  ATTN_HIP,
  ATTN_GENERIC,
  ATTN_ASM,
};
enum AttnItem {
  ATTN_ITEM_512,
  ATTN_ITEM_256,
};
inline int attn_item_wave_rows(AttnItem item) { return item == ATTN_ITEM_512 ? 128 : 64; }
struct AttnAsmLaunch {
  int64_t rows = 0;
  AttnItem item = ATTN_ITEM_512;
  bool grouped = false;
};
struct AttnPlan {
  AttnFamily family = ATTN_HIP;
  int hd_index = 0;
  int planes = 1;
  AttnAsmLaunch main, tail;
};
int f3r_attn_plan(const f3r_attn_args& a, AttnPlan* plan);
bool f3r_attn_asm_plan(const f3r_attn_args& a, int64_t min_keys, AttnPlan* plan, const char** why);
int f3r_attn_asm_launch(const f3r_attn_args& a, const AttnPlan& plan, hipStream_t stream);
const char* f3r_attn_asm_name(const f3r_attn_args& a, const AttnPlan& plan);
int f3r_attn_generic_launch(const f3r_attn_args& a, hipStream_t stream);
```

fast3r_amd/csrc/f3r_gemm_asm.hip:

```cpp
#include <cstddef>
#include <cstring>

#include "f3r_common.h"
#include "f3r_dispatch.h"

extern "C" const unsigned char f3r_gemm_asm_hsaco[];
extern "C" const unsigned int f3r_gemm_asm_hsaco_len;

namespace {

struct f3r_gemm_asm_args {
  const void* A;
  const void* W;
  const float* bias;
  const float* res;
  void* out;
  uint32_t lda_b, ldw_b, ldr_b, ldo_b;
  uint32_t nk, nk1;
  uint32_t xq, xr, pg, pg_magic, gm_shift, act, grid, n_wg;
  int64_t seg_stride;
  uint32_t tps, tps_magic;
  float scale;
  uint32_t flags, nk1_w, pad;
  const uint32_t* w_scale;
  uint32_t nk8, out8_off;
  const float* rope_cos;
  const float* rope_sin;
  uint32_t seq_len, seq_magic, rope_w, rope_w_magic;
};
static_assert(sizeof(f3r_gemm_asm_args) == 176 && offsetof(f3r_gemm_asm_args, w_scale) == 128 && offsetof(f3r_gemm_asm_args, rope_cos) == 144 && offsetof(f3r_gemm_asm_args, lda_b) == 40 && offsetof(f3r_gemm_asm_args, xq) == 64 &&
              offsetof(f3r_gemm_asm_args, seg_stride) == 96 && offsetof(f3r_gemm_asm_args, nk1_w) == 120, "must match ARG_* of gemm_gen.py");
enum { ACT_SCALE = 3, ACT_ROPE = 4, FLAG_BIAS_ON_M = 1, FLAG_SKEW = 2 };

enum { ROLE_F32 = 0, ROLE_LP = 1 };
F3rCodeObject<6> g_kernels = {f3r_gemm_asm_hsaco, {"f3r_gemm_asm_f32_f16", "f3r_gemm_asm_f32_bf16", "f3r_gemm_asm_lp_f16", "f3r_gemm_asm_lp_bf16", "f3r_gemm_asm_f328_f16", "f3r_gemm_asm_lp8_f16"}};

hipFunction_t get_fn(int role, int dtype, bool f8 = false) {
  if (dtype < 0 || dtype > 1 || (f8 && dtype != F3R_F16)) return nullptr;
  return g_kernels.get(f8 ? 4 + role : 2 * role + dtype);
}

int role_of(const f3r_gemm_args& a) { return a.out_f32 ? ROLE_F32 : ROLE_LP; }

bool one_output_eligible(const f3r_gemm_args& a, const char** why) {
  if (a.out_f32 && a.out_lp) { *why = "both an fp32 and a lowp output"; return false; }
  if (a.out_f32) {
    if (a.act != F3R_ACT_NONE) { *why = "activation on the fp32 role"; return false; }
    if ((a.ldo_f32 * 4) % 16 != 0 || (a.res_f32 && (a.ldr_f32 * 4) % 16 != 0)) { *why = "fp32 row strides not multiples of 16 bytes"; return false; }
    if ((int64_t)256 * a.ldo_f32 * 4 >= (1ll << 32) || (a.res_f32 && (int64_t)256 * a.ldr_f32 * 4 >= (1ll << 32))) { *why = "fp32 row strides too large"; return false; }
  } else {
    if (a.res_f32) { *why = "fp32 residual with a lowp output"; return false; }
    if ((((uintptr_t)a.out_lp) & 15) != 0 || (a.ldo_lp * 2) % 16 != 0) { *why = "lowp output not 16-byte aligned"; return false; }
    if ((int64_t)256 * a.ldo_lp * 2 >= (1ll << 32)) { *why = "lowp row stride too large"; return false; }
  }
  return true;
}

}

static uint32_t gm_shift(int64_t ntm) {
  uint32_t gsh = 3;
  while (ntm % (1ll << gsh)) --gsh;
  return gsh;
}
static bool tile_map_exact(int64_t ntm, int64_t ntn, int64_t tps) {
  const int64_t n_wg = ntm * ntn, pg = (1ll << gm_shift(ntm)) * ntn;
  return n_wg * pg < (1ll << 32) && ntn * (tps > 0 ? tps : 1) < (1ll << 32);
}

bool f3r_gemm_asm_preferred(int64_t tiles) {
  const int64_t cus = f3r_num_cus();
  if (tiles < cus) return false;
  const int64_t rounds = (tiles + cus - 1) / cus;
  return tiles * 5 >= rounds * cus * 4;
}

bool f3r_gemm_asm_eligible(const f3r_gemm_args& a, const char** why) {
  *why = "";
  if (a.a_mode != F3R_A_PLAIN) { *why = "not a plain GEMM operand (convolution)"; return false; }
  if (a.epi != F3R_EPI_GENERIC) { *why = "QKV / ConvT epilogue"; return false; }
  if (a.split != F3R_SPLIT_NONE && a.split != F3R_SPLIT_W2) { *why = "X3 split"; return false; }
  if (a.M <= 0 || a.M % 256 != 0 || a.N % 256 != 0) { *why = "M or N not a multiple of 256"; return false; }
  const int Kpad1 = a.split ? a.Kpad / 2 : a.Kpad;
  if (a.K != Kpad1 || Kpad1 % 64 != 0) { *why = "K is not the padded depth (a K tail cannot be zero-filled by LDS-DMA)"; return false; }
  if ((a.Kpad / 64) < 4) { *why = "fewer than 4 K-tiles (the operand streams run three K-tiles ahead)"; return false; }
  if (a.rowadd || a.res_lp || a.res_lp2 || a.out_lp_lo || a.out_relu || a.out_relu_lo || a.out_f8 || a.out_relu_f8 || a.fin_w) { *why = "additive rows / lowp residuals / second outputs"; return false; }
  if (!one_output_eligible(a, why)) return false;
  if ((int64_t)256 * a.lda * 2 >= (1ll << 32) || (int64_t)256 * a.Kpad * 2 >= (1ll << 32)) { *why = "operand row strides too large for 32-bit lane offsets"; return false; }
  const int64_t tiles = (a.M / 256) * (a.N / 256);
  if (tiles >= (1ll << 24)) { *why = "grid too large"; return false; }
  if (!tile_map_exact(a.M / 256, a.N / 256, a.N / 256)) { *why = "tile map: position x period reaches 2^32 (the kernel divides by multiplying with ceil(2^32 / period))"; return false; }
  if (get_fn(role_of(a), a.dtype) == nullptr) { *why = "the embedded code object could not be loaded on this device"; return false; }
  return true;
// ... 60 lines not shown
  f3r_gemm_asm_args k;
  memset(&k, 0, sizeof(k));
  k.A = a.A;
  k.W = a.W;
  k.bias = a.bias;
  k.res = role == ROLE_F32 ? a.res_f32 : nullptr;
  k.out = role == ROLE_F32 ? (void*)a.out_f32 : a.out_lp;
  k.lda_b = (uint32_t)(a.lda * 2);
  k.ldr_b = (uint32_t)(a.ldr_f32 * 4);
  k.ldo_b = role == ROLE_F32 ? (uint32_t)(a.ldo_f32 * 4) : (uint32_t)(a.ldo_lp * 2);
  fill_k_loop(k, a, f8);
  k.act = (uint32_t)a.act;
  k.scale = 1.0f;
  k.out8_off = (f8 && a.out_lp_f8) ? (uint32_t)a.N * 2u : 0u;
  return launch_tiles(fn, k, a.M, a.N, stream, plan.skew, role);
}

bool f3r_gemm_asm_f8_eligible(const f3r_gemm_args& a, const char** why) {
  *why = "";
  if (a.dtype != F3R_F16) { *why = "the fp8 low plane corrects fp16 planes only"; return false; }
  if (a.a_mode != F3R_A_PLAIN || a.epi != F3R_EPI_GENERIC) { *why = "not a plain GEMM with the generic epilogue"; return false; }
  if (a.M <= 0 || a.M % 256 != 0 || a.N % 256 != 0) { *why = "M or N not a multiple of 256"; return false; }
  if (a.K % 128 != 0 || a.K / 64 + a.K / 128 < 4) { *why = "K not a multiple of 128, or fewer than 4 K-tiles"; return false; }
  if (a.rowadd || a.res_lp || a.res_lp2 || a.out_lp_lo || a.out_relu || a.out_relu_lo || a.A_lo) { *why = "additive rows / lowp residuals / second outputs / A_lo"; return false; }
  if (!one_output_eligible(a, why)) return false;
  if (!a.out_f32 && a.out_lp_f8 && (a.act != F3R_ACT_GELU || a.ldo_lp * 2 < (int64_t)a.N * 3)) { *why = "out_lp_f8 needs the GELU epilogue and rows of >= 3 N / 2 elements"; return false; }
  if (a.out_lp_f8 && a.out_f32) { *why = "out_lp_f8 with an fp32 output"; return false; }
  if ((int64_t)256 * a.lda * 2 >= (1ll << 32) || (int64_t)256 * a.K * 3 >= (1ll << 32)) { *why = "operand row strides too large for 32-bit lane offsets"; return false; }
  if ((a.M / 256) * (int64_t)(a.N / 256) >= (1ll << 24) || !tile_map_exact(a.M / 256, a.N / 256, a.N / 256)) { *why = "grid too large"; return false; }
  if (get_fn(role_of(a), a.dtype, true) == nullptr) { *why = "the embedded code object could not be loaded on this device"; return false; }
  return true;
}

bool f3r_gemm_asm_qkv_eligible(const f3r_gemm_args& a, const char** why) {
  *why = "";
  if (a.epi != F3R_EPI_QKV || a.a_mode != F3R_A_PLAIN) { *why = "not a QKV launch"; return false; }
  if (a.rope_cos) {
    if (a.rope_mode != 0 || a.rope_w <= 0) { *why = "rotary embedding per row group (rope_mode 1)"; return false; }
    if (a.M * (int64_t)a.seq_len >= (1ll << 32) || (int64_t)a.seq_len * a.rope_w >= (1ll << 32)) { *why = "token index x sequence length reaches 2^32 (magic-number division)"; return false; }
  }
  if (a.split != F3R_SPLIT_NONE && a.split != F3R_SPLIT_W2 && a.split != F3R_SPLIT_W2F8) { *why = "X3 split"; return false; }
  const bool f8 = a.split == F3R_SPLIT_W2F8;
  if (f8 && (a.dtype != F3R_F16 || !a.w_scale || !a.W_aux || a.K % 128 != 0 || a.Kpad != a.K)) { *why = "W2F8 needs fp16, w_scale, W_aux, K = Kpad a multiple of 128"; return false; }
  const int Dq = a.qkv_dq ? a.qkv_dq : a.N / 3;
  const int Dkv = (a.N - Dq) / 2;
  if (Dq != Dkv) { *why = "grouped-query widths (q and k segments differ)"; return false; }
  if (Dq % 256 != 0 || a.M <= 0 || a.M % 256 != 0 || a.seq_len % 256 != 0) { *why = "D, M or seq_len not a multiple of 256"; return false; }
  const int Kpad1 = (a.split && !f8) ? a.Kpad / 2 : a.Kpad;
  if (a.K != Kpad1 || Kpad1 % 64 != 0 || a.Kpad / 64 < 4) { *why = "K tail or fewer than 4 K-tiles"; return false; }
  if ((((uintptr_t)a.q) & 15) || (((uintptr_t)a.k) & 15) || (((uintptr_t)a.vt) & 15) || (a.ldvt * 2) % 16 != 0) { *why = "outputs not 16-byte aligned"; return false; }
  if ((int64_t)256 * a.lda * 2 >= (1ll << 32) || (int64_t)256 * a.Kpad * 3 >= (1ll << 32) || (int64_t)256 * a.ldvt * 2 >= (1ll << 32)) { *why = "row strides too large"; return false; }
  if ((a.M / 256) * (int64_t)(a.N / 256) >= (1ll << 24)) { *why = "grid too large"; return false; }
  if (!tile_map_exact(a.M / 256, 2 * (Dq / 256), Dq / 256) || !tile_map_exact(Dq / 256, a.M / 256, a.seq_len / 256)) { *why = "tile map: position x period reaches 2^32"; return false; }
  if (get_fn(ROLE_LP, a.dtype) == nullptr || (f8 && get_fn(ROLE_LP, a.dtype, true) == nullptr)) { *why = "the embedded code object could not be loaded on this device"; return false; }
  return true;
}

static int qkv_launch(const f3r_gemm_args& a, hipStream_t stream, bool skew) {
  const bool f8 = a.split == F3R_SPLIT_W2F8;
  hipFunction_t fn = get_fn(ROLE_LP, a.dtype), fn_qk = f8 ? get_fn(ROLE_LP, a.dtype, true) : fn;
  if (!fn || !fn_qk) return not_loaded();
  const int D = a.qkv_dq ? a.qkv_dq : a.N / 3;
  f3r_gemm_asm_args k;
  memset(&k, 0, sizeof(k));
  k.A = a.A;
  k.W = a.W;
  k.bias = a.bias;
  k.out = a.q;
  k.lda_b = (uint32_t)(a.lda * 2);
  k.ldo_b = (uint32_t)(D * 2);
  fill_k_loop(k, a, f8);
  k.act = a.rope_cos ? ACT_ROPE : ACT_SCALE;
  k.scale = a.q_scale != 0.f ? a.q_scale : 1.0f;
  if (a.rope_cos) {
    k.rope_cos = a.rope_cos;
    k.rope_sin = a.rope_sin;
    k.seq_len = (uint32_t)a.seq_len;
    k.seq_magic = a.seq_len > 1 ? (uint32_t)(((1ull << 32) + (uint64_t)a.seq_len - 1) / (uint64_t)a.seq_len) : 0;
    k.rope_w = (uint32_t)a.rope_w;
    k.rope_w_magic = a.rope_w > 1 ? (uint32_t)(((1ull << 32) + (uint64_t)a.rope_w - 1) / (uint64_t)a.rope_w) : 0;
  }
  k.seg_stride = (int64_t)((const char*)a.k - (const char*)a.q);
  k.tps = (uint32_t)(D / 256);
  int rc = launch_tiles(fn_qk, k, a.M, 2 * (int64_t)D, stream, skew, ROLE_LP);
  if (rc != F3R_OK) return rc;
  f3r_gemm_asm_args v;
  memset(&v, 0, sizeof(v));
  const int64_t kp_v = f8 ? (int64_t)2 * a.K : a.Kpad;
  v.A = f8 ? a.W_aux : (const void*)((const char*)a.W + (int64_t)2 * D * a.Kpad * 2);
  v.W = a.A;
  v.bias = a.bias ? a.bias + 2 * D : nullptr;
  v.out = a.vt;
  v.lda_b = (uint32_t)(kp_v * 2);
  v.ldw_b = (uint32_t)(a.lda * 2);
  v.ldo_b = (uint32_t)(a.ldvt * 2);
  v.nk = f8 ? (uint32_t)(2 * (a.K / 64)) : k.nk;
  v.nk1 = v.nk;
  v.nk1_w = f8 ? (uint32_t)(a.K / 64) : k.nk1;
  v.scale = 1.0f;
  v.flags = FLAG_BIAS_ON_M;
  v.seg_stride = (int64_t)D * a.ldvt * 2;
  v.tps = (uint32_t)(a.seq_len / 256);
  return launch_tiles(fn, v, D, a.M, stream, skew, ROLE_LP);
}
```

fast3r_amd/fast3r.py:

```python
import math
import time
from collections import OrderedDict
from copy import deepcopy

from typing import NamedTuple, Optional

import numpy as np
import torch
import torch.nn as nn

from . import dpt_head, ops
from ._lib import F3RError
from .dist import ViewSharding, split_range
from .packing import _f32, _pack_block, _pack_dino_block, _pack_llama_block
from .params import (_ROPE_PERM, CroCoEncoder, DinoEncoder, Fast3RDecoder, LlamaDecoder, PixelwiseTaskWithDPT,
                     sincos_1d_table)


class OperandFormat(NamedTuple):
    lp: torch.dtype
    planes: bool
    low_f8: bool
    fc1_planes: bool
    head_f8: bool
    linear_split: Optional[str]
    x3: bool
    qk3: bool
    qk3_planes: int
    qk3_encoder: bool
    head_f8_min_rows: int
    head_tail_fused_min_rows: int

    @property
    def pack_part(self):
        return self[:5]


def _fills_chip(rows, cols):
    return (rows // 256) * (cols // 256) >= 256


def _planes(fmt, x_f32):
    if fmt.planes:
        return ops.cast_lp(x_f32, fmt.lp, want_lo=True)
    return ops.cast_lp(x_f32, fmt.lp), None


def _f8_gemms(pb, T, seq_len):
    qk = (pb.qk_w8 is not None and T % 256 == 0 and seq_len % 256 == 0 and pb.rope_mode == 0 and pb.q_dim == 0
          and _fills_chip(T, pb.qk_w8.shape[0]))
    fc1 = pb.fc1_w8 is not None and T % 256 == 0 and not pb.swiglu_hidden and _fills_chip(T, pb.fc1_w8.shape[0])
    return qk, fc1, fc1 and _fills_chip(T, pb.fc2_w8.shape[0])


class _GraphCache:

    def __init__(self):
        self.max_views = 64
        self.max_entries = 8
        self.entries = OrderedDict()
        self.seen = set()

    def clear(self):
        self.entries.clear()
        self.seen.clear()

    def run(self, model, views, host_outputs=False):
        imgs = [v["img"] for v in views]
        dev = imgs[0].device
        shapes = {tuple(i.shape) for i in imgs}
        if len(views) > self.max_views or len(shapes) != 1 or any(i.dtype != torch.float32 for i in imgs):
            return None
        if model._orientation_plan(views)["any_portrait"]:
            return None
        key = (len(views), tuple(imgs[0].shape), str(dev), model.max_parallel_views_for_head, model.training, model._params_version(), model._format())
        dec = model.decoder
        B = imgs[0].shape[0]
        if key not in self.entries:
            if key not in self.seen:
                self.seen.add(key)
                return None
            static_imgs = [torch.empty_like(i) for i in imgs]
            static_emb = torch.zeros((B, len(views), dec.embed_dim), dtype=torch.float32, device=dev)
            static_views = [{"img": t} for t in static_imgs]
            for t, i in zip(static_imgs, imgs):
                t.copy_(i)
            graph = torch.cuda.CUDAGraph()
            sched = torch.zeros(2, dtype=torch.int32, device=dev)
            torch.cuda.synchronize()
            with torch.cuda.graph(graph), ops.sched_scope(sched):
                outs = model._forward_eager(static_views, False, _emb_rows=static_emb)
            self.entries[key] = (graph, static_imgs, static_emb, outs, sched)
            while len(self.entries) > self.max_entries:
                self.entries.popitem(last=False)
        self.entries.move_to_end(key)
        graph, static_imgs, static_emb, outs, _sched = self.entries[key]
        for t, i in zip(static_imgs, imgs):
            t.copy_(i, non_blocking=True)
        ids = dec.draw_image_ids(B, len(views))
        static_emb.copy_(dec.image_idx_emb.to(dev)[ids.to(dev)])
        graph.replay()
        if host_outputs:
            sink = _HostSink(dev, B)
            sink.push([(i, slice(None), k, v) for i, r in enumerate(outs) for k, v in r.items()], [])
            sink.finish()
# ... 278 lines not shown
    @property
    def _head_f8(self):
        return self._format().head_f8

    def _pack(self, device, fmt=None):
        fmt = fmt or self._format()
        lp, hp = fmt.lp, fmt.planes
        key = (str(device), self._params_version(), fmt.pack_part)
        if self._packed is not None and self._packed["key"] == key:
            return self._packed
        alt = getattr(self, "_packed_alt", None)
        if alt is not None and alt["key"] == key:
            self._packed, self._packed_alt = alt, self._packed
            return self._packed
        if self._packed is not None and self._packed["key"][1] != key[1]:
            self._packed = self._packed_alt = None
            self._graphs.clear()
        if alt is not None:
            self._graphs.clear()
        self._packed_alt = self._packed
        enc, dec = self.encoder, self.decoder
        pk = dict(key=key)
        dino = isinstance(enc, DinoEncoder)
        vit = enc.model if dino else enc
        norm = vit.norm if dino else enc.enc_norm
        pk["pe_w"] = ops.pack_linear_weight(vit.patch_embed.proj.weight.detach().float(), lp, hp)
        pk["pe_b"] = _f32(vit.patch_embed.proj.bias)
        pk["enc"] = [_pack_dino_block(b, lp, hp) for b in vit.blocks] if dino else [_pack_block(b, fmt) for b in enc.enc_blocks]
        pk["enc_norm"] = (_f32(norm.weight), _f32(norm.bias), norm.eps)
        if dino:
            pk["dino_pos"] = {}
        pk["de_w"] = ops.pack_linear_weight(dec.decoder_embed.weight.detach().float(), lp, hp)
        pk["de_b"] = _f32(dec.decoder_embed.bias)
        if isinstance(dec, LlamaDecoder):
            pk["dec"] = [_pack_llama_block(b, dec.num_heads, lp, hp, dec.n_kv_heads, dec.is_causal) for b in dec.layers]
            pk["dec_norm"] = (_f32(dec.norm.weight), None, dec.norm.eps)
            pk["view0"] = _f32(dec.view0_embed)
        else:
            pk["dec"] = [_pack_block(b, fmt, dec.embed_dim // dec.num_heads) for b in dec.dec_blocks]
            pk["dec_norm"] = (_f32(dec.dec_norm.weight), _f32(dec.dec_norm.bias), dec.dec_norm.eps)
        pk["head"] = dpt_head._pack_head(self.downstream_head, fmt)
        pk["head_local"] = dpt_head._pack_head(self.downstream_head_local, fmt) if self.downstream_head_local is not None else None
        self._packed = pk
        return pk

    def _rope(self, n_pos, device):
        key = (n_pos, str(device))
        if key not in self._rope_cache:
            self._rope_cache[key] = ops.rope_tables(n_pos, self.encoder.rope_freq, device)
        return self._rope_cache[key]

    def _block_ws(self, fmt, pb, T, D, n_seq, seq_len, dev, external_kv=False):
        hidden = pb.fc1_w.shape[0]
        f8_rows = any(_f8_gemms(pb, T, seq_len))
        return ops.BlockWorkspace(T, D, hidden, n_seq, seq_len, fmt.lp, dev, kv_dim=0 if external_kv else pb.kv_dim, f8_rows=f8_rows)

    def _block(self, fmt, x, pb, n_heads, scale, seq_len, n_seq, rope, kv_exchange=None, ws=None, kv_tap=None):
        lp, sp = fmt.lp, fmt.linear_split
        if fmt.x3:
            return self._block_exact(fmt, x, pb, n_heads, scale, seq_len, n_seq, rope, kv_exchange)
        D = x.shape[1]
        T = x.shape[0]
        if ws is None:
            ws = self._block_ws(fmt, pb, T, D, n_seq, seq_len, x.device)
        q = ws.q
        if kv_exchange is None:
            k, vt = ws.k, ws.vt
            ldvt = vt.shape[-1]
        else:
            k, vt = kv_exchange.k_loc, kv_exchange.vt_loc
        f8_qkv, f8_fc1, f8_fc2 = _f8_gemms(pb, T, seq_len)
        if f8_qkv:
            rows1 = ops.layernorm_f8(x, pb.n1w, pb.n1b, pb.eps, out_rows=ws.rows8(D), rms=pb.rms)
            ops.gemm_qkv(rows1, pb.qk_w8, pb.qkv_b, q, k, vt, seq_len, rope, q_scale=scale * ops.LOG2E, split="w2f8", w_scale=pb.qk_ws, w_aux=pb.v_w2)
            h = ws.h
        else:
            h, _ = ops.layernorm(x, pb.n1w, pb.n1b, pb.eps, lp, out_lp=ws.h, rms=pb.rms)
            ops.gemm_qkv(h, pb.qkv_w, pb.qkv_b, q, k, vt, seq_len, rope, q_scale=scale * ops.LOG2E, rope_mode=pb.rope_mode, split=sp, q_dim=pb.q_dim)
        if kv_tap is not None and kv_exchange is None:
            kv_tap(k, vt)
        o = h
        gqa = dict(kv_group=pb.kv_group, causal=pb.causal, head_dim=pb.head_dim)
        if kv_exchange is None:
            Dkv = k.shape[1]
            ops.attention(q, o, n_heads, scale, [(k, vt, seq_len, seq_len * Dkv, Dkv * ldvt)], tq=seq_len, batch=n_seq,
                          q_batch_stride=seq_len * D, o_batch_stride=seq_len * D, q_prescaled=True, **gqa)
        else:
            sharding = self.sharding
            sharding.begin_layer(kv_exchange)
            kv_exchange.start()
            if seq_len == 0:
                kv_exchange.finish()
            elif kv_exchange.has_remote:
                pos = kv_exchange.positions()
                ops.attention(q, o, n_heads, scale, [kv_exchange.local_segment()], tq=seq_len, q_prescaled=True,
                              state=kv_exchange.state, state_out=True, q_pos0=pos[kv_exchange.rank], seg_pos0=[pos[kv_exchange.rank]],
                              reserve_cus=getattr(sharding, "reserve_cus", 0), **gqa)
                kv_exchange.mark_local_done()
                groups = [(w, sg) for w, sg in kv_exchange.remote_groups()]
                live = [i for i, (_, sg) in enumerate(groups) if sg]
                for i, (wait, segs) in enumerate(groups):
                    wait()
                    if live and i == live[0]:
                        kv_exchange.mark_remote_start()
                    if not segs:
                        continue
                    ops.attention(q, o, n_heads, scale, segs, tq=seq_len, q_prescaled=True, state=kv_exchange.state, state_in=True,
                                  state_out=(i != live[-1]), q_pos0=pos[kv_exchange.rank],
                                  seg_pos0=[kv_exchange.remote_position_of(sg) for sg in segs], **gqa)
            else:
                kv_exchange.finish()
                ops.attention(q, o, n_heads, scale, [kv_exchange.local_segment()], tq=seq_len, q_prescaled=True, **gqa)
            sharding.end_layer(kv_exchange)
        ops.gemm(o, pb.proj_w, bias=pb.proj_b, res_f32=x, out_f32=x, split=sp)
        if f8_fc1:
            rows = ops.layernorm_f8(x, pb.n2w, pb.n2b, pb.eps, out_rows=ws.rows8(D), rms=pb.rms)
            if f8_fc2:
                _, hid = ops.gemm(rows, pb.fc1_w8, bias=pb.fc1_b, act="gelu", out_lp=ws.hid8(), split="w2f8", w_scale=pb.fc1_ws, out_f8_rows=True)
                ops.gemm(hid, pb.fc2_w8, bias=pb.fc2_b, res_f32=x, out_f32=x, split="w2f8", w_scale=pb.fc2_ws)
            else:
                _, hid = ops.gemm(rows, pb.fc1_w8, bias=pb.fc1_b, act="gelu", out_lp=ws.hid, split="w2f8", w_scale=pb.fc1_ws)
                ops.gemm(hid, pb.fc2_w, bias=pb.fc2_b, res_f32=x, out_f32=x, split=sp)
            return x
        h2, _ = ops.layernorm(x, pb.n2w, pb.n2b, pb.eps, lp, out_lp=o, rms=pb.rms)
        if pb.swiglu_hidden:
            _, ab = ops.gemm(h2, pb.fc1_w, out_lp=ws.hid, split=sp)
            hid = ops.silu_mul(ab, pb.swiglu_hidden)
        else:
            _, hid = ops.gemm(h2, pb.fc1_w, bias=pb.fc1_b, act="gelu", out_lp=ws.hid, split=sp if pb.fc1_split in (None, True) else None)
        ops.gemm(hid, pb.fc2_w, bias=pb.fc2_b, res_f32=x, out_f32=x, split=sp)
        return x

    def _block_exact(self, fmt, x, pb, n_heads, scale, seq_len, n_seq, rope, kv_exchange):
        lp = fmt.lp
        T = x.shape[0]
        _, hf = ops.layernorm(x, pb.n1w, pb.n1b, pb.eps, lp, want_lp=False, want_f32=True, rms=pb.rms)
        h, hl = _planes(fmt, hf)
        qkv, _ = ops.gemm(h, pb.qkv_w, bias=pb.qkv_b, want_f32=True, split="x3", a_lo=hl)
        n_kv = n_heads // pb.kv_group
        if rope is not None and T:
            ops.rope_f32(qkv, n_heads + n_kv, max(1, seq_len), rope, pb.rope_mode)
        gqa = dict(head_dim=pb.head_dim, kv_group=pb.kv_group, causal=pb.causal)
        if kv_exchange is None and fmt.qk3 and self._qk3_ok(fmt, pb, n_seq, seq_len) and (n_seq == 1 or fmt.qk3_encoder):
            planes = fmt.qk3_planes
            qp, kp, vt = ops.qkv_planes(qkv, n_heads, n_kv, n_seq, seq_len, scale * ops.LOG2E, lp, planes=planes)
            state = ops.attention_state(T, n_heads, x.device, pb.head_dim)
            ldvt_ = vt.shape[-1]
            ops.attention(qp, state[0], n_heads, scale, [(kp, vt.view(n_seq * n_kv * 64, ldvt_), seq_len, seq_len * n_kv * 128, n_kv * 64 * ldvt_)], tq=seq_len,
                          batch=n_seq, q_batch_stride=seq_len * n_heads * 128, o_batch_stride=seq_len * n_heads * 64, q_prescaled=True, state=state,
                          state_out=True, kv_group=pb.kv_group, head_dim=64, qk_planes=planes, kernel_sel=2)
            o, ol = ops.attention_state_finish(state, n_heads, 64, lp)
            del qp, kp, vt, state
        elif kv_exchange is None:
            o, ol = ops.attention_f32(qkv, n_heads, n_seq, seq_len, scale, lp, **gqa)
        else:
            Dq, Dkv = n_heads * pb.head_dim, n_kv * pb.head_dim
            k_all, v_all = kv_exchange.gather_rows_f32(qkv[:, Dq:Dq + Dkv], qkv[:, Dq + Dkv:])
            if T:
                o, ol = ops.attention_f32(qkv, n_heads, 1, seq_len, scale, lp, kv=(k_all, v_all), q_pos0=kv_exchange.positions()[kv_exchange.rank], **gqa)
            else:
                o = ol = torch.empty((0, Dq), dtype=lp, device=x.device)
        ops.gemm(o, pb.proj_w, bias=pb.proj_b, res_f32=x, out_f32=x, split="x3", a_lo=ol)
        _, hf = ops.layernorm(x, pb.n2w, pb.n2b, pb.eps, lp, want_lp=False, want_f32=True, out_f32=hf, rms=pb.rms)
        h, hl = _planes(fmt, hf)
        if pb.swiglu_hidden:
            ab, _ = ops.gemm(h, pb.fc1_w, want_f32=True, split="x3", a_lo=hl)
            hid, hid_lo = ops.silu_mul_f32(ab, pb.swiglu_hidden, lp)
# ... 356 lines not shown
```

fast3r_amd/ops.py:

```python
import ctypes
import math

import torch

from . import _lib
from ._lib import (AttnArgs, F3R_A_CONV3X3, F3R_A_PLAIN, F3R_ACT_GELU, F3R_ACT_NONE, F3R_ACT_RELU, F3R_EPI_CONVT,
                   F3R_EPI_GENERIC, F3R_EPI_QKV, F3R_MAX_SEG, F3R_SPLIT_NONE, F3R_SPLIT_W2, F3R_SPLIT_W2F8, F3R_SPLIT_X3, F3R_SPLIT_X3F8, GemmArgs, check, dtype_id,
                   ptr, require_gpu, stream_ptr)

ACT = {None: F3R_ACT_NONE, "none": F3R_ACT_NONE, "gelu": F3R_ACT_GELU, "relu": F3R_ACT_RELU}

ATTN_TIMER = None
ATTN_COUNTERS = None
ATTN_WORK_STEALING = True
_SCHED = {}
_SCHED_CAPTURE = None


class sched_scope:

    def __init__(self, counter):
        assert counter.dtype == torch.int32 and counter.numel() >= 2 and counter.is_cuda
        self.counter = counter

# ... 263 lines not shown
    g.dtype = dtype_id(lp)
    if w_scale is not None:
        g.w_scale = ptr(w_scale)
    g.out_lp_f8 = int(bool(out_f8_rows))
    with _timed(2.0 * M * N * K):
        check(_lib.lib().f3r_gemm(ctypes.byref(g), stream_ptr()), "f3r_gemm")
    if out_lp_lo is not None:
        return out_f32, out_lp, out_lp_lo
    return out_f32, out_lp


class BlockWorkspace:

    def __init__(self, tokens, D, hidden, n_seq, seq_len, lp, device, kv_dim=None, f8_rows=False):
        kv_dim = D if kv_dim is None else kv_dim
        offs = (ctypes.c_size_t * 5)()
        f8_rows = bool(f8_rows) and lp == torch.float16 and D % 8 == 0 and hidden % 8 == 0
        total = _lib.lib().f3r_block_workspace_bytes_ex(tokens, D, kv_dim, hidden, n_seq, seq_len, int(f8_rows), offs)
        if total == 0:
            raise ValueError(f"f3r_block_workspace_bytes: bad sizes ({tokens=}, {D=}, {hidden=}, {n_seq=}, {seq_len=})")
        self.buf = torch.empty((total,), dtype=torch.uint8, device=device)
        ld = vt_ld(seq_len)

        def view(i, shape, wide=False):
            n = 1
            for d in shape:
                n *= d
            return self.buf[offs[i]:offs[i] + 2 * n].view(lp).view(shape)
        self.h, self.q, self.k = view(0, (tokens, D)), view(1, (tokens, D)), view(2, (tokens, kv_dim))
        self.vt, self.hid = view(3, (n_seq, kv_dim, ld)), view(4, (tokens, hidden))
        if ld != seq_len and kv_dim:
            self.vt.zero_()
        self.key = (tokens, D, hidden, n_seq, seq_len, lp, str(device))
        self._rows8 = view(0, (tokens, 3 * D // 2)) if f8_rows else None
        self._hid8 = view(4, (tokens, 3 * hidden // 2)) if f8_rows else None

    def hid8(self):
        if self._hid8 is None:
            self._hid8 = torch.empty((self.hid.shape[0], 3 * self.hid.shape[1] // 2), dtype=torch.float16, device=self.buf.device)
        return self._hid8

    def rows8(self, D):
        if self._rows8 is None:
            self._rows8 = torch.empty((self.h.shape[0], 3 * D // 2), dtype=torch.float16, device=self.buf.device)
        assert self._rows8.shape[1] == 3 * D // 2
        return self._rows8


def vt_ld(seq_len: int) -> int:
    return round_up(seq_len, 64)


LOG2E = 1.4426950408889634


def gemm_qkv(a, w, bias, q, k, vt, seq_len, rope=None, q_scale=0.0, rope_mode=0, split=None, a_lo=None, kernel_sel=0, q_dim=0, w_scale=None, w_aux=None):
    require_gpu(a, "a")
    lp = a.dtype
    M = a.shape[0]
    N, Kpad = w.shape
    K = a.shape[1]
    if split == "w2f8":
        assert w_scale is not None and w_aux is not None and lp == torch.float16 and w_aux.dtype == lp
        K = Kpad = 2 * w.shape[1] // 3
        N = w.shape[0] + w_aux.shape[0]
        assert w_aux.shape[1] == 2 * K and a.shape[1] * 2 >= 3 * K and w_scale.numel() == w.shape[0]
    g = GemmArgs()
    g.A, g.W, g.bias = ptr(a), ptr(w), ptr(bias)
    g.M, g.N, g.K, g.Kpad, g.lda = M, N, K, Kpad, a.stride(0)
    if split == "w2f8":
        g.w_scale, g.W_aux = ptr(w_scale), ptr(w_aux)
    g.a_mode, g.epi, g.act = F3R_A_PLAIN, F3R_EPI_QKV, F3R_ACT_NONE
    g.q, g.k, g.vt = ptr(q), ptr(k), ptr(vt)
    g.seq_len, g.ldvt = seq_len, vt.stride(-2)
    if rope is not None:
        g.rope_cos, g.rope_sin, g.rope_w = ptr(rope[0]), ptr(rope[1]), rope[2]
        g.rope_mode = int(rope_mode)
    g.q_scale = float(q_scale)
    g.qkv_dq = int(q_dim)
    g.kernel_sel = kernel_sel
    _split_operand(g, a, split, a_lo)
    g.dtype = dtype_id(lp)
    with _timed(2.0 * M * N * K):
        check(_lib.lib().f3r_gemm(ctypes.byref(g), stream_ptr()), "f3r_gemm(qkv)")


def silu_mul(ab, hidden, out=None):
    require_gpu(ab, "ab")
    assert ab.dim() == 2 and ab.shape[1] == 2 * hidden and ab.is_contiguous()
    if out is None:
        out = torch.empty((ab.shape[0], hidden), dtype=ab.dtype, device=ab.device)
    with _timed(0.0, _nb(ab, out), "elementwise"):
        check(_lib.lib().f3r_silu_mul(ptr(ab), ptr(out), ab.shape[0], hidden, dtype_id(ab.dtype), stream_ptr()), "f3r_silu_mul")
    return out


def rows_add(x, vec, rows):
    require_gpu(x, "x")
    assert x.dtype == torch.float32 and x.is_contiguous() and vec.dtype == torch.float32 and vec.numel() == x.shape[-1]
    check(_lib.lib().f3r_rows_add_f32(ptr(x), ptr(vec), int(rows), x.shape[-1], stream_ptr()), "f3r_rows_add_f32")
    return x


def conv3x3(x, w, *, stride=1, bias=None, a_relu=False, act=None, res_lp=None, res_lp2=None, out=None, split=None, x_lo=None,
            res_lp_lo=None, res_lp2_lo=None, want_lo=False, want_relu=False, kernel_sel=0, x_f8=None, w_scale=None, want_f8=False,
            want_relu_lo=None, want_relu_f8=False, fin=None):
    require_gpu(x, "x")
    lp = x.dtype
    assert x.is_contiguous() and x.dim() == 4
    B, H, W, C = x.shape
    OH, OW = (H + 2 - 3) // stride + 1, (W + 2 - 3) // stride + 1
    N, Kpad = w.shape
    g = GemmArgs()
    g.kernel_sel = kernel_sel
    if split == "x3f8":
        assert x_f8 is not None and x_f8.dtype == torch.uint8 and x_f8.shape == (B, H, W, 2 * C) and x_f8.is_contiguous() and w_scale is not None
        g.split, g.A_lo, g.w_scale = F3R_SPLIT_X3F8, ptr(x_f8), ptr(w_scale)
    else:
        _split_operand(g, x, split, x_lo)
    extra = {}
    pts = conf = None
    if fin is not None:
        fw, fb, n_out, dmode, cmode, vmin, vmax, want_conf = fin
        assert fw.dtype == torch.float32 and fw.shape == (4, N) and fw.is_contiguous() and fb.dtype == torch.float32 and fb.numel() == 4
# ... 25 lines not shown
        g.res_lp_lo = ptr(res_lp_lo)
    if res_lp2_lo is not None:
        g.res_lp2_lo = ptr(res_lp2_lo)
    g.A, g.W, g.bias = ptr(x), ptr(w), ptr(bias)
    g.M, g.N, g.K, g.Kpad, g.lda = B * OH * OW, N, 0, Kpad, 0
    g.a_mode, g.a_relu = F3R_A_CONV3X3, int(a_relu)
    g.conv_H, g.conv_W, g.conv_C, g.conv_stride, g.conv_OH, g.conv_OW = H, W, C, stride, OH, OW
    g.epi, g.act = F3R_EPI_GENERIC, ACT[act]
    if res_lp is not None:
        g.res_lp, g.ldr_lp = ptr(res_lp), N
    if res_lp2 is not None:
        g.res_lp2, g.ldr_lp2 = ptr(res_lp2), N
    g.dtype = dtype_id(lp)
    with _timed(2.0 * B * OH * OW * N * 9 * C + (8.0 * B * OH * OW * N if fin is not None else 0.0)):
        check(_lib.lib().f3r_gemm(ctypes.byref(g), stream_ptr()), "f3r_gemm(conv3x3)")
    if fin is not None:
        return pts, conf
    if extra:
        extra["out"] = out
        return extra
    return out


def convT(x, w, bias_tiled, s, cout, split=None, x_lo=None, want_lo=False, kernel_sel=0):
    require_gpu(x, "x")
    lp = x.dtype
    B, h, wd, cin = x.shape
    out = torch.empty((B, h * s, wd * s, cout), dtype=lp, device=x.device)
    g = GemmArgs()
    g.kernel_sel = kernel_sel
    _split_operand(g, x, split, x_lo)
    out_lo = None
    if want_lo:
        out_lo = torch.empty_like(out)
        g.out_lp_lo = ptr(out_lo)
    g.A, g.W, g.bias = ptr(x), ptr(w), ptr(bias_tiled)
    g.M, g.N, g.K, g.Kpad, g.lda = B * h * wd, s * s * cout, cin, w.shape[1], cin
    g.a_mode, g.epi, g.act = F3R_A_PLAIN, F3R_EPI_CONVT, F3R_ACT_NONE
    g.out_lp, g.ldo_lp = ptr(out), cout
    g.ct_s, g.ct_h, g.ct_w, g.ct_cout = s, h, wd, cout
    g.dtype = dtype_id(lp)
    with _timed(2.0 * B * h * wd * s * s * cout * cin):
        check(_lib.lib().f3r_gemm(ctypes.byref(g), stream_ptr()), "f3r_gemm(convT)")
    return (out, out_lo) if want_lo else out


def attention_state(tq_total: int, n_heads: int, device, head_dim: int = 64):
    return (torch.empty((tq_total, n_heads * head_dim), dtype=torch.float32, device=device),
            torch.empty((tq_total, n_heads, 4), dtype=torch.float32, device=device))


def attention(q, out, n_heads, scale, segments, tq=None, batch=1, q_batch_stride=0, o_batch_stride=0, q_prescaled=False,
              state=None, state_in=False, state_out=False, kv_group=1, causal=False, q_pos0=0, seg_pos0=None, kernel_sel=0, head_dim=64, qk_planes=1,
              reserve_cus=0):
    require_gpu(q, "q")
    lp = q.dtype
    assert 1 <= len(segments) <= F3R_MAX_SEG
    a = AttnArgs()
    a.q, a.o = ptr(q), ptr(out)
    a.ldq, a.ldo = q.stride(-2), out.stride(-2)
    a.q_batch_stride, a.o_batch_stride = q_batch_stride, o_batch_stride
    a.tq = q.shape[-2] if tq is None else tq
    a.batch, a.n_heads, a.n_seg, a.dtype = batch, n_heads, len(segments), dtype_id(lp)
    for i, (k, vt, seg_len, kbs, vbs) in enumerate(segments):
        assert k.dtype == lp and vt.dtype == lp
        a.k_seg[i], a.vt_seg[i] = ptr(k), ptr(vt)
        a.seg_len[i], a.ldvt[i] = seg_len, vt.stride(-2)
        a.k_batch_stride[i], a.vt_batch_stride[i] = kbs, vbs
        a.ldk = k.stride(-2)
    a.scale = float(scale)
    a.q_prescaled = int(q_prescaled)
    a.kv_group, a.causal, a.q_pos0 = int(kv_group), int(bool(causal)), int(q_pos0)
    a.kernel_sel = int(kernel_sel)
    a.head_dim = int(head_dim)
    a.qk_planes = int(qk_planes)
    a.reserve_cus = int(reserve_cus)
    if causal:
        pos = [0] * len(segments)
        if seg_pos0 is None:
            run = 0
            for i, sgm in enumerate(segments):
                pos[i] = run
                run += int(sgm[2])
        else:
            pos = [int(v) for v in seg_pos0]
        for i, v in enumerate(pos):
            a.seg_pos0[i] = v
    if ATTN_COUNTERS is not None:
        assert ATTN_COUNTERS.dtype == torch.int32 and ATTN_COUNTERS.numel() >= 56 and ATTN_COUNTERS.data_ptr() % 8 == 0 and ATTN_COUNTERS.device == q.device
        a.dbg_counters = ptr(ATTN_COUNTERS)
    if state is not None:
        a.st_o, a.st_ml = ptr(state[0]), ptr(state[1])
        a.state_in, a.state_out = int(state_in), int(state_out)
    if ATTN_WORK_STEALING:
        a.sched_counter = ptr(_sched_counter(q.device))
    if ATTN_TIMER is not None:
        e0, e1 = torch.cuda.Event(enable_timing=True), torch.cuda.Event(enable_timing=True)
        e0.record()
    with _timed(4.0 * a.tq * sum(int(s_[2]) for s_ in segments) * head_dim * n_heads * batch, 0.0, "attention"):
        check(_lib.lib().f3r_attn_fwd(ctypes.byref(a), stream_ptr()), "f3r_attn_fwd")
    if ATTN_TIMER is not None:
        e1.record()
        t_k = sum(int(s[2]) for s in segments)
        ATTN_TIMER.append((e0, e1, 4.0 * a.tq * t_k * head_dim * n_heads * batch, int(a.tq), int(t_k),
                           _lib.lib().f3r_attn_kernel_name(ctypes.byref(a)).decode()))
    return out


def qkv_planes(qkv, n_heads, kv_heads, n_seq, seq_len, q_scale, lp, planes=2):
    require_gpu(qkv, "qkv")
    assert qkv.dtype == torch.float32 and qkv.dim() == 2 and qkv.stride(1) == 1 and qkv.shape[0] == n_seq * seq_len
    T = qkv.shape[0]
    qp = torch.empty((T, n_heads * 128), dtype=lp, device=qkv.device)
    kp = torch.empty((T, kv_heads * 128), dtype=lp, device=qkv.device)
    ld = vt_ld(seq_len)
    vt = torch.empty((n_seq, kv_heads * 64, ld), dtype=lp, device=qkv.device)
    with _timed(0.0, _nb(qkv, qp, kp, vt), "elementwise"):
        check(_lib.lib().f3r_qkv_planes(ptr(qkv), qkv.stride(0), n_seq, seq_len, n_heads, kv_heads, float(q_scale), ptr(qp), ptr(kp), ptr(vt), ld, dtype_id(lp),
                                        int(planes), stream_ptr()), "f3r_qkv_planes")
    return qp, kp, vt


def attention_state_finish(state, n_heads, head_dim, lp, want_lo=True, want_f32=False):
    st_o, st_ml = state
    require_gpu(st_o, "st_o")
    T, D = st_o.shape[0], n_heads * head_dim
    assert st_o.shape == (T, D) and st_ml.shape == (T, n_heads, 4) and st_o.is_contiguous() and st_ml.is_contiguous()
    o_hi = torch.empty((T, D), dtype=lp, device=st_o.device)
    o_lo = torch.empty((T, D), dtype=lp, device=st_o.device) if want_lo else None
    o32 = torch.empty((T, D), dtype=torch.float32, device=st_o.device) if want_f32 else None
    with _timed(0.0, _nb(st_o, st_ml, o_hi, o_lo, o32), "elementwise"):
        check(_lib.lib().f3r_attn_state_finish(ptr(st_o), ptr(st_ml), T, n_heads, head_dim, ptr(o_hi), ptr(o_lo), ptr(o32), D, dtype_id(lp), stream_ptr()),
              "f3r_attn_state_finish")
    return (o_hi, o_lo, o32) if want_f32 else (o_hi, o_lo)


def upsample2x(x, out_hw=None, x_lo=None, want_lo=False, want_f8=False):
    B, h, w, C = x.shape
    oh, ow = (2 * h, 2 * w) if out_hw is None else out_hw
    return interp_bilinear(x, (oh, ow), x_lo=x_lo, want_lo=want_lo, want_f8=want_f8, nominal_hw=(2 * h, 2 * w))


DEPTH_MODES = {"exp": 0, "linear": 1, "square": 2}
CONF_MODES = {"exp": 0, "sigmoid": 1}


def interp_bilinear(x, full_hw, x_lo=None, want_lo=False, want_f8=False, nominal_hw=None):
    require_gpu(x, "x")
    B, h, w, C = x.shape
    oh, ow = full_hw
    fh, fw = (oh, ow) if nominal_hw is None else nominal_hw
    out = torch.empty((B, oh, ow, C), dtype=x.dtype, device=x.device)
    out_lo = torch.empty_like(out) if want_lo else None
# ... 117 lines not shown
```

fast3r_amd/packing.py:

```python
import torch

from . import ops
from .params import _ROPE_PERM, _Block, _DinoBlock, _LlamaBlock


class _PackedBlock:
    __slots__ = ("n1w", "n1b", "n2w", "n2b", "eps", "qkv_w", "qkv_b", "proj_w", "proj_b", "fc1_w", "fc1_b", "fc2_w", "fc2_b",
                 "rms", "rope_mode", "swiglu_hidden", "q_dim", "kv_dim", "kv_group", "causal", "head_dim", "fc1_split",
                 "fc1_w8", "fc1_ws", "fc2_w8", "fc2_ws",
                 "qk_w8", "qk_ws", "v_w2")

    def __init__(self, norm1, norm2):
        self.n1w, self.n1b, self.n2w, self.n2b = (_f32(getattr(n, a, None)) for n in (norm1, norm2) for a in ("weight", "bias"))
        self.eps = norm1.eps
        self.fc1_w8 = self.fc1_ws = self.fc2_w8 = self.fc2_ws = self.qk_w8 = self.qk_ws = self.v_w2 = None
        self.rms, self.rope_mode, self.swiglu_hidden = False, 0, 0
        self.fc1_split = None
        self.head_dim = 64
        self.q_dim, self.kv_dim, self.kv_group, self.causal = 0, None, 1, False


def _f32(t):
    return None if t is None else t.detach().float().contiguous()


def _pack_block(blk: _Block, fmt, head_dim=64):
    p = _PackedBlock(blk.norm1, blk.norm2)
    lp, split = fmt.lp, fmt.planes
    p.head_dim = head_dim
    p.qkv_w, p.qkv_b = ops.pack_linear_weight(blk.attn.qkv.weight.detach().float(), lp, split), _f32(blk.attn.qkv.bias)
    p.proj_w, p.proj_b = ops.pack_linear_weight(blk.attn.proj.weight.detach().float(), lp, split), _f32(blk.attn.proj.bias)
    p.fc1_split = fmt.fc1_planes
    p.fc1_w, p.fc1_b = ops.pack_linear_weight(blk.mlp.fc1.weight.detach().float(), lp, p.fc1_split), _f32(blk.mlp.fc1.bias)
    p.fc2_w, p.fc2_b = ops.pack_linear_weight(blk.mlp.fc2.weight.detach().float(), lp, split), _f32(blk.mlp.fc2.bias)
    w1 = blk.mlp.fc1.weight.detach().float()
    w2_ = blk.mlp.fc2.weight.detach().float()
    if fmt.low_f8 and p.fc1_split and w1.shape[1] % 128 == 0 and w1.shape[0] % 256 == 0 and w2_.shape[0] % 256 == 0:
        p.fc1_w8, p.fc1_ws = ops.pack_linear_weight_f8(w1)
        p.fc2_w8, p.fc2_ws = ops.pack_linear_weight_f8(w2_)
    wq = blk.attn.qkv.weight.detach().float()
    Dm = wq.shape[0] // 3
    if fmt.low_f8 and wq.shape[1] % 128 == 0 and Dm % 256 == 0 and head_dim == 64:
        p.qk_w8, p.qk_ws = ops.pack_linear_weight_f8(wq[:2 * Dm])
        p.v_w2 = ops.pack_linear_weight(wq[2 * Dm:], lp, True)
    return p


def _pack_dino_block(blk: _DinoBlock, lp, split=False):
    p = _PackedBlock(blk.norm1, blk.norm2)
    g1, g2 = blk.ls1.gamma.detach().float(), blk.ls2.gamma.detach().float()
    p.qkv_w, p.qkv_b = ops.pack_linear_weight(blk.attn.qkv.weight.detach().float(), lp, split), _f32(blk.attn.qkv.bias)
    p.proj_w = ops.pack_linear_weight(g1[:, None] * blk.attn.proj.weight.detach().float(), lp, split)
    p.proj_b = (g1 * blk.attn.proj.bias.detach().float()).contiguous()
    p.fc1_w, p.fc1_b = ops.pack_linear_weight(blk.mlp.fc1.weight.detach().float(), lp, split), _f32(blk.mlp.fc1.bias)
    p.fc2_w = ops.pack_linear_weight(g2[:, None] * blk.mlp.fc2.weight.detach().float(), lp, split)
    p.fc2_b = (g2 * blk.mlp.fc2.bias.detach().float()).contiguous()
    return p


def _pack_llama_block(blk: _LlamaBlock, n_heads, lp, split=False, n_kv_heads=None, causal=False):
    p = _PackedBlock(blk.attention_norm, blk.ffn_norm)
    p.rms, p.rope_mode = True, 1
    n_kv_heads = n_heads if n_kv_heads is None else n_kv_heads
    perm = torch.tensor([h * 64 + d for h in range(n_heads) for d in _ROPE_PERM])
    perm_kv = torch.tensor([h * 64 + d for h in range(n_kv_heads) for d in _ROPE_PERM])
    wq, wk, wv = (m.weight.detach().float() for m in (blk.attention.wq, blk.attention.wk, blk.attention.wv))
    p.qkv_w, p.qkv_b = ops.pack_linear_weight(torch.cat([wq[perm], wk[perm_kv], wv], dim=0), lp, split), None
    if n_kv_heads != n_heads:
        p.q_dim, p.kv_dim, p.kv_group = n_heads * 64, n_kv_heads * 64, n_heads // n_kv_heads
    p.causal = bool(causal)
    p.proj_w, p.proj_b = ops.pack_linear_weight(blk.attention.wo.weight.detach().float(), lp, split), None
    w1, w3 = blk.feed_forward.w1.weight.detach().float(), blk.feed_forward.w3.weight.detach().float()
    p.swiglu_hidden = w1.shape[0]
    p.fc1_w, p.fc1_b = ops.pack_linear_weight(torch.cat([w1, w3], dim=0), lp, split), None
    p.fc2_w, p.fc2_b = ops.pack_linear_weight(blk.feed_forward.w2.weight.detach().float(), lp, split), None
    return p
```

include/f3r.h:

```cpp
#ifndef F3R_H_
#define F3R_H_

#include <stddef.h>
#include <stdint.h>

#ifdef __cplusplus
extern "C" {
#endif

typedef void* f3r_stream_t;

typedef enum {
  F3R_OK = 0,
  F3R_ERR_ARG = -1,
  F3R_ERR_UNSUPPORTED = -2,
  F3R_ERR_LAUNCH = -3
} f3r_status;

typedef enum { F3R_F16 = 0, F3R_BF16 = 1 } f3r_dtype;
typedef enum { F3R_REAL_F32 = 0, F3R_REAL_F64 = 1 } f3r_real;
typedef enum { F3R_LOSS_DIS = 0, F3R_LOSS_LOG1P = 1 } f3r_loss_dis_mode;

#define F3R_MAX_SEG 8

// ... 21 lines not shown
  int32_t N;
  int32_t K;
  int32_t Kpad;
  int64_t lda;
  int32_t a_mode;
  int32_t a_relu;
  int32_t conv_H, conv_W, conv_C, conv_stride, conv_OH, conv_OW;
  int32_t epi;
  int32_t act;
  const float* rowadd;
  int64_t rowadd_div;
  const float* res_f32;
  int64_t ldr_f32;
  const void* res_lp;
  int64_t ldr_lp;
  const void* res_lp2;
  int64_t ldr_lp2;
  float* out_f32;
  int64_t ldo_f32;
  void* out_lp;
  int64_t ldo_lp;
  void* q;
  void* k;
  void* vt;
  int64_t seq_len;
  int64_t ldvt;
  const float* rope_cos;
  const float* rope_sin;
  int32_t rope_w;
  float q_scale;
  int32_t ct_s, ct_h, ct_w, ct_cout;
  int32_t dtype;
  int32_t rope_mode;
  int32_t split;
  int32_t kernel_sel;
  const void* A_lo;
  void* out_lp_lo;
  const void* res_lp_lo;
  const void* res_lp2_lo;
  void* out_relu;
  void* out_relu_lo;
  int32_t qkv_dq;
  int32_t out_lp_f8;
  const uint32_t* w_scale;
  const void* W_aux;
  void* out_f8;
  void* out_relu_f8;
  const float* fin_w;
  const float* fin_b;
  float* fin_pts;
  float* fin_conf;
  int32_t fin_n_out, fin_depth_mode, fin_conf_mode;
  float fin_vmin, fin_vmax;
  int32_t reserved0;
} f3r_gemm_args;

typedef enum { F3R_SPLIT_NONE = 0, F3R_SPLIT_W2 = 1, F3R_SPLIT_X3 = 2, F3R_SPLIT_W2F8 = 3, F3R_SPLIT_X3F8 = 4 } f3r_split;

int f3r_gemm(const f3r_gemm_args* args, f3r_stream_t stream);

size_t f3r_block_workspace_bytes(int64_t tokens, int D, int kv_dim, int hidden, int64_t n_seq, int64_t seq_len, size_t offsets[5]);
size_t f3r_block_workspace_bytes_ex(int64_t tokens, int D, int kv_dim, int hidden, int64_t n_seq, int64_t seq_len, int f8_rows, size_t offsets[5]);

typedef struct f3r_attn_args {
  const void* q;
  void* o;
  int64_t ldq, ldo;
  int64_t q_batch_stride, o_batch_stride;
  int64_t tq;
  int32_t batch;
  int32_t n_heads;
  int32_t n_seg;
  int32_t dtype;
  const void* k_seg[F3R_MAX_SEG];
  const void* vt_seg[F3R_MAX_SEG];
  int64_t seg_len[F3R_MAX_SEG];
  int64_t ldvt[F3R_MAX_SEG];
  int64_t ldk;
  int64_t k_batch_stride[F3R_MAX_SEG];
  int64_t vt_batch_stride[F3R_MAX_SEG];
  float scale;
  int32_t q_prescaled;
  float* st_o;
  float* st_ml;
  int32_t state_in;
  int32_t state_out;
  int32_t kv_group;
  int32_t causal;
  int64_t q_pos0;
  int64_t seg_pos0[F3R_MAX_SEG];
  int32_t kernel_sel;
  int32_t head_dim;
  uint32_t* dbg_counters;
  uint32_t* sched_counter;
  int32_t qk_planes;
  int32_t reserve_cus;
} f3r_attn_args;
#define F3R_ATTN_ASM_MIN_KEYS 2048
#define F3R_ATTN_GROUPED_MIN_KEYS 8192

int f3r_attn_fwd(const f3r_attn_args* args, f3r_stream_t stream);
const char* f3r_attn_kernel_name(const f3r_attn_args* args);

int f3r_upsample2x(const void* in, const void* in_lo, void* out, void* out_lo, int batch, int h, int w, int C, int out_h, int out_w,
                   int dtype, f3r_stream_t stream);
int f3r_interp_bilinear(const void* in, const void* in_lo, void* out, void* out_lo, int batch, int h, int w, int C, int full_h, int full_w,
                        int out_h, int out_w, int dtype, f3r_stream_t stream);
int f3r_interp_bilinear_f8(const void* in, const void* in_lo, void* out, void* out_lo, void* out_f8, int batch, int h, int w, int C, int full_h,
                           int full_w, int out_h, int out_w, int dtype, f3r_stream_t stream);

typedef enum { F3R_DEPTH_EXP = 0, F3R_DEPTH_LINEAR = 1, F3R_DEPTH_SQUARE = 2 } f3r_depth_mode;
typedef enum { F3R_CONF_EXP = 0, F3R_CONF_SIGMOID = 1 } f3r_conf_mode;
int f3r_dpt_final(const void* x, const void* x_lo, const float* w, const float* b, int n_out, float* pts3d, float* conf, int64_t npix,
                  int Cin, int depth_mode, int conf_mode, float conf_vmin, float conf_vmax, int dtype, f3r_stream_t stream);

int f3r_cast_f32_to_lp(const float* in, void* out, void* out_lo, int64_t n, int dtype, f3r_stream_t stream);

size_t f3r_align_workspace_bytes(int n_prob);
int f3r_align_local_to_global(const float* conf, const float* pts_local, const float* pts_global, const uint8_t* valid_mask,
                              float* out, float* rts, float* thr_out, void* workspace, size_t ws_bytes, int n_prob,
                              int64_t npix, float quantile, f3r_stream_t stream);

size_t f3r_focal_workspace_bytes(int n_views, int H, int W);
int f3r_estimate_focal(const float* pts3d, const float* conf, float* focal, float* thr_out, void* workspace, size_t ws_bytes,
                       int n_views, int H, int W, float quantile, float ppx, float ppy, int n_iter, float min_focal, float max_focal,
                       f3r_stream_t stream);

size_t f3r_nn_index_bytes(int64_t m);
size_t f3r_nn_workspace_bytes(int64_t n);
int f3r_nn_build(const float* pts, int64_t m, void* index, size_t index_bytes, void* workspace, size_t ws_bytes, f3r_stream_t stream);
int f3r_nn_query(const void* index, const float* query, int64_t n, double* dist, int32_t* idx, void* workspace, size_t ws_bytes,
                 f3r_stream_t stream);
int f3r_estimate_normals(const void* index, const float* pts, int k, double* normals, int32_t* knn_idx, double* knn_dist, f3r_stream_t stream);
size_t f3r_recon_stats_workspace_bytes(int64_t n);
int f3r_recon_stats(const double* dist, const int32_t* idx, const double* normals_q, const double* normals_db, int64_t n, int64_t m_db,
                    double dist_th, double* out, void* workspace, size_t ws_bytes, f3r_stream_t stream);
size_t f3r_recon_prepare_workspace_bytes(int n_samples, int n_views, int64_t L);
int f3r_recon_prepare(const float* conf, const float* pred, const float* gt, const uint8_t* valid, const int64_t* seg, int n_samples,
                      int n_views, int64_t L, float q_metric, float q_icp, float* pred_out, float* gt_out, int32_t* counts, float* rts,
                      void* workspace, size_t ws_bytes, f3r_stream_t stream);

int f3r_estimate_poses(const float* pts3d, const float* conf, const float* focal_in, float* focal_out, float* cam_to_world, int* inliers,
                       int n_views, int H, int W, float conf_thr, float ppx, float ppy, int n_focals, int n_iter, f3r_stream_t stream);

int f3r_pose_pair_metrics(const void* pred, const void* gt, int dtype, int n_samples, int n_views, const double* r_thresholds, int n_r,
                          const double* t_thresholds, int n_t, int n_bins, double max_threshold, void* rel_r, void* rel_t, int64_t* counts,
                          f3r_stream_t stream);
int f3r_pose_error_stats(const void* r, const void* t, int64_t n, int dtype, const double* r_thresholds, int n_r, const double* t_thresholds,
                         int n_t, int n_bins, double max_threshold, int64_t* counts, f3r_stream_t stream);

size_t f3r_mv_conf_loss_workspace_bytes(int n_views, int n_samples);
int f3r_mv_conf_loss(const void* const* gt_pts, const void* const* valid_mask, const void* const* camera_pose, int pose_dtype,
                     const void* const* pred_pts, const void* const* pred_conf, const void* const* pred_pts_local,
                     const void* const* pred_conf_local, const int64_t* n_pixels, int n_views, int n_samples, int version, int dis_mode,
                     int gt_scale, int local_scale_consistent, int use_dist_clip, double dist_clip, double alpha, void* workspace,
// ... 188 lines not shown
```

Baseline: 36.36.

## Write e4m3 copy of attention output and run proj and V GEMMs in fp8-split mode

The hand-written attention kernels gain an o8 variant that also stores a clamped e4m3 copy of the output next to the fp16 one, in the fp8 row workspace. That lets the attention projection GEMM run in the w2f8 split mode with fp8-packed weights instead of the plain fp16 path. The V part of the QKV weight is also packed as fp8 with per-row scales, and a GEMM variant with the scale taken on the A side is generated. The aim is to raise MFMA throughput and reduce the bytes the proj and V GEMMs read. In exchange it adds extra stores and conversions to the attention epilogue and relies on the split-precision scheme to keep accuracy.

Measured after the change: 36.54 (median of 6 runs). Within noise of the previous version (+0.5%).

```diff
diff --git a/fast3r_amd/_lib.py b/fast3r_amd/_lib.py
--- a/fast3r_amd/_lib.py
+++ b/fast3r_amd/_lib.py
@@ -59,7 +59,7 @@
         ("w_scale", _c_vp), ("W_aux", _c_vp),
         ("out_f8", _c_vp), ("out_relu_f8", _c_vp),
         ("fin_w", _c_vp), ("fin_b", _c_vp), ("fin_pts", _c_vp), ("fin_conf", _c_vp),
-        ("fin_n_out", _c_i32), ("fin_depth_mode", _c_i32), ("fin_conf_mode", _c_i32), ("fin_vmin", _c_f32), ("fin_vmax", _c_f32), ("reserved0", _c_i32),
+        ("fin_n_out", _c_i32), ("fin_depth_mode", _c_i32), ("fin_conf_mode", _c_i32), ("fin_vmin", _c_f32), ("fin_vmax", _c_f32), ("w_aux_f8", _c_i32),
     ]
 
 
@@ -106,6 +106,7 @@
     "f3r_gemm": (ctypes.c_int, [ctypes.POINTER(GemmArgs), _c_vp]),
     "f3r_attn_fwd": (ctypes.c_int, [ctypes.POINTER(AttnArgs), _c_vp]),
     "f3r_attn_kernel_name": (ctypes.c_char_p, [ctypes.POINTER(AttnArgs)]),
+    "f3r_attn_fwd_o8": (ctypes.c_int, [ctypes.POINTER(AttnArgs), ctypes.c_uint32, _c_vp]),
     "f3r_block_workspace_bytes": (ctypes.c_size_t, [_c_i64, ctypes.c_int, ctypes.c_int, ctypes.c_int, _c_i64, _c_i64, ctypes.POINTER(ctypes.c_size_t)]),
     "f3r_block_workspace_bytes_ex": (ctypes.c_size_t, [_c_i64, ctypes.c_int, ctypes.c_int, ctypes.c_int, _c_i64, _c_i64, ctypes.c_int, ctypes.POINTER(ctypes.c_size_t)]),
     "f3r_upsample2x": (ctypes.c_int, [_c_vp, _c_vp, _c_vp, _c_vp, ctypes.c_int, ctypes.c_int, ctypes.c_int, ctypes.c_int, ctypes.c_int, ctypes.c_int, ctypes.c_int, _c_vp]),
@@ -230,6 +231,7 @@
 SYMBOL_IF_PRESENT_MATCH = frozenset(name for name in SYMBOLS if name.startswith("f3r_match_"))
 SYMBOL_IF_PRESENT_CLEAN = frozenset(name for name in SYMBOLS if name.startswith("f3r_clean_"))
 SYMBOL_IF_PRESENT_GALIGN = frozenset(name for name in SYMBOLS if name.startswith("f3r_galign_"))
+SYMBOL_IF_PRESENT_ATTN_O8 = frozenset(("f3r_attn_fwd_o8",))
 
 
 def symbol_since(name: str) -> int:
@@ -237,7 +239,7 @@
 
 
 def if_present(name: str) -> bool:
-    return (name in SYMBOL_IF_PRESENT or name in SYMBOL_IF_PRESENT_MAPS or name in SYMBOL_IF_PRESENT_VIEWS or name in SYMBOL_IF_PRESENT_DEPTH
+    return (name in SYMBOL_IF_PRESENT_ATTN_O8 or name in SYMBOL_IF_PRESENT or name in SYMBOL_IF_PRESENT_MAPS or name in SYMBOL_IF_PRESENT_VIEWS or name in SYMBOL_IF_PRESENT_DEPTH
             or name in SYMBOL_IF_PRESENT_MATCH or name in SYMBOL_IF_PRESENT_CLEAN or name in SYMBOL_IF_PRESENT_GALIGN)
 
 
diff --git a/fast3r_amd/csrc/asm/attn_gen.py b/fast3r_amd/csrc/asm/attn_gen.py
--- a/fast3r_amd/csrc/asm/attn_gen.py
+++ b/fast3r_amd/csrc/asm/attn_gen.py
@@ -14,6 +14,7 @@
 ARG_KBS = 80
 ARG_STLD = 96
 ARG_TQ = 104
+ARG_O8OFF = 108
 ARG_SEG = 112
 SEG_BYTES = 24
 ARG_DBG = ARG_SEG + 8 * SEG_BYTES
@@ -53,8 +54,10 @@
 
 class AttnGen:
     def __init__(self, dtype="f16", rowsum="pkadd", big_gap=None, k8_gap=2, name=None, ablate=(), cvt="rne", dma_aux="", dma_start=8, dma_step=None, pf=None, nslot=4,
-                 fold="dot", head_dim=64, qk_planes=1, corr="f16", qk3_queues=True, k_hoist=True, qpw=None, tiles_per_barrier=1):
+                 fold="dot", head_dim=64, qk_planes=1, corr="f16", qk3_queues=True, k_hoist=True, qpw=None, tiles_per_barrier=1, o8=False):
         assert dtype in ("f16", "bf16")
+        assert not o8 or (dtype == "f16" and head_dim == 64 and qk_planes == 1), "the fp8 copy of O: head_dim 64, fp16, one product"
+        self.o8 = bool(o8)
         assert head_dim in (64, 80, 128), "head widths with a generated kernel"
         assert qk_planes in (1, 2) and (qk_planes == 1 or (head_dim == 64 and dtype == "f16")) and corr in ("f16", "f8") and (corr == "f16" or qk_planes == 2)
         self.qk_planes, self.corr = qk_planes, corr
@@ -141,6 +144,8 @@
         self.name = name or (f"f3r_attn_asm_q256_{dtype}" if (D == 64 and qk_planes == 1 and self.QPW == 2) else f"f3r_attn_asm_qk3f8_{dtype}" if corr == "f8" else f"f3r_attn_asm_qk3_{dtype}" if qk_planes == 2 else f"f3r_attn_asm_{dtype}" if D == 64 else f"f3r_attn_asm_d{D}_{dtype}")
         if name is None and G > 1:
             self.name += "_grp"
+        if name is None and self.o8:
+            self.name += "_o8"
         self.p = Program(self.name)
         if dtype == "f16":
             self.MFMA, self.MFMA8 = "v_mfma_f32_32x32x16_f16", "v_mfma_f32_32x32x8_f16"
@@ -868,11 +873,27 @@
         e("v_xor_b32", V(7), 32, V(LANE))
         e("v_lshlrev_b32", V(7), 2, V(7), comment="(lane ^ 32) * 4")
         e("s_lshl_b32", S(47), s_ldo, 5)
+        SETW = 6
+        if self.o8:
+            SETW = 8
+            s_o8 = S(48, 2)
+            e("s_load_dword", S(50), S(0, 2), Lit(ARG_O8OFF))
+            e("s_lshl_b32", S(51), S(3), 6, comment="head * 64 bytes")
+            e("s_mov_b32", S(44), Lit(0x43E00000), comment="448.0: the largest e4m3 number (v_cvt_pk_fp8_f32 makes NaN of anything larger)")
+            e("s_mov_b32", S(45), Lit(0xC3E00000), comment="-448.0")
+            e("v_lshlrev_b32", V(5), 2, V(3))
+            e("v_sub_u32", V(8), V(4), V(5), comment="lq * ldo + g * 4")
+            e("s_waitcnt", "lgkmcnt(0)")
+            e("s_sub_u32", S(50), S(50), S(51))
+            e("s_add_u32", s_o8.sub(0), s_o.sub(0), S(50))
+            e("s_addc_u32", s_o8.sub(1), s_o.sub(1), 0)
         k = 0
         for qb in range(self.QPW):
             if qb:
                 e("s_mov_b64", EXEC, -1)
                 e("v_add_u32", V(4), S(47), V(4))
+                if self.o8:
+                    e("v_add_u32", V(8), S(47), V(8))
             e("ds_bpermute_b32", V(5), V(7), V(self.LRUN + qb))
             e("s_waitcnt", "lgkmcnt(0)")
             e("v_add_f32", V(5), V(5), V(self.LRUN + qb))
@@ -880,7 +901,7 @@
             self.own_rows_mask(qb)
             for db in range(self.NDB):
                 for rq in self.rq_range(db):
-                    t = 16 + 6 * (k % 4)
+                    t = 16 + SETW * (k % 4)
                     k += 1
                     if k > 4 and (k - 1) % 4 == 0:
                         e("s_waitcnt", "vmcnt(0)")
@@ -891,6 +912,14 @@
                     e(self.CVT, V(t + 4), V(t), V(t + 1))
                     e(self.CVT, V(t + 5), V(t + 2), V(t + 3))
                     e("global_store_dwordx2", V(4), V(t + 4, 2), s_o, offset=db * 64 + rq * 16)
+                    if self.o8:
+                        for i in range(4):
+                            e("v_max_f32", V(t + i), S(45), V(t + i))
+                        for i in range(4):
+                            e("v_min_f32", V(t + i), S(44), V(t + i))
+                        e("v_cvt_pk_fp8_f32", V(t + 6), V(t), V(t + 1))
+                        e("v_cvt_pk_fp8_f32", V(t + 6), V(t + 2), V(t + 3), text="op_sel:[0,0,1]")
+                        e("global_store_dword", V(8), V(t + 6), s_o8, offset=db * 32 + rq * 8)
         self.item_done()
         self.lab("STATE_OUT")
         self.state_rows_offsets()
@@ -1191,6 +1220,15 @@
     return gens
 
 
+def o8_generators(**kw):
+    gens = []
+    for extra in (dict(), dict(qpw=2), dict(GROUPED_RING)):
+        g = AttnGen("f16", head_dim=64, o8=True, **dict(kw, **extra))
+        g.build()
+        gens.append(g)
+    return gens
+
+
 def main():
     import argparse
     ap = argparse.ArgumentParser()
@@ -1219,6 +1257,7 @@
         a.pf, a.nslot = None, 4
     gens = product_generators(ring=ring, rowsum=a.rowsum, big_gap=bg, k8_gap=a.k8_gap, ablate=[x for x in a.ablate.split(",") if x], cvt=a.cvt,
                               dma_aux=a.dma_aux, dma_start=a.dma_start, dma_step=a.dma_step, pf=a.pf, nslot=a.nslot, fold=a.fold, qk3_queues=bool(a.qk3_queues), k_hoist=bool(a.k_hoist))
+    gens += o8_generators()
     for g in gens:
         problems = g.p.check_hazards() if not a.ablate else []
         if problems:
diff --git a/fast3r_amd/csrc/asm/gemm_gen.py b/fast3r_amd/csrc/asm/gemm_gen.py
--- a/fast3r_amd/csrc/asm/gemm_gen.py
+++ b/fast3r_amd/csrc/asm/gemm_gen.py
@@ -92,14 +92,15 @@
 
 
 class GemmGen:
-    def __init__(self, dtype="f16", role="f32", name=None, ablate=(), f8=False):
+    def __init__(self, dtype="f16", role="f32", name=None, ablate=(), f8=False, scale_rows="w"):
         assert dtype in ("f16", "bf16") and role in ("f32", "lp")
         assert not (f8 and dtype != "f16"), "the fp8 low plane corrects fp16 planes (the split modes are an fp16 design)"
-        self.dtype, self.role, self.f8 = dtype, role, f8
+        assert scale_rows in ("w", "a") and (scale_rows == "w" or (f8 and role == "lp"))
+        self.dtype, self.role, self.f8, self.scale_rows = dtype, role, f8, scale_rows
         self.perm = role == "lp"
         self.esize = 4 if role == "f32" else 2
         self.ablate = set(ablate)
-        self.name = name or f"f3r_gemm_asm_{role}{'8' if f8 else ''}_{dtype}"
+        self.name = name or f"f3r_gemm_asm_{role}{'8' if f8 else ''}{'a' if scale_rows == 'a' else ''}_{dtype}"
         self.arg_size = ARG_SIZE_LP if role == "lp" else (ARG_SIZE_F8 if f8 else ARG_SIZE)
         self.MFMA8 = "v_mfma_scale_f32_32x32x64_f8f6f4"
         self.lds_bytes = LDS_BYTES
@@ -176,8 +177,12 @@
 
     def wsc_ptr(self):
         e = self.e
-        e("s_lshl_b32", T[3], s_wn, 7)
-        e("s_add_u32", T[3], T[3], T[9], comment="first output column of this wave")
+        if self.scale_rows == "a":
+            e("s_lshl_b32", T[3], s_wm, 7)
+            e("s_add_u32", T[3], T[3], T[8], comment="first output row of this wave")
+        else:
+            e("s_lshl_b32", T[3], s_wn, 7)
+            e("s_add_u32", T[3], T[3], T[9], comment="first output column of this wave")
         e("s_lshl_b32", T[4], T[3], 2)
         e("s_add_u32", s_wsc.sub(0), s_argWsc.sub(0), T[4])
         e("s_addc_u32", s_wsc.sub(1), s_argWsc.sub(1), 0)
@@ -330,6 +335,9 @@
 
     def mfmas8(self, q):
         ks, pair = q // 2, q % 2
+        if self.scale_rows == "a":
+            return [self.I(self.MFMA8, ACC(2 * pair + x, j), W8(q % 2, x), A8(ks % 2, j), ACC(2 * pair + x, j), V(VUNIT), V(SCW + j), text="op_sel_hi:[0,0,0]")
+                    for x in range(2) for j in range(4)]
         return [self.I(self.MFMA8, ACC(2 * pair + x, j), W8(q % 2, x), A8(ks % 2, j), ACC(2 * pair + x, j), V(SCW + 2 * pair + x), V(VUNIT), text="op_sel_hi:[0,0,0]")
                 for x in range(2) for j in range(4)]
 
@@ -1111,6 +1119,9 @@
         g = GemmGen("f16", role, f8=True, **kw)
         g.build()
         gens.append(g)
+    g = GemmGen("f16", "lp", f8=True, scale_rows="a", **kw)
+    g.build()
+    gens.append(g)
     return gens
 
 
diff --git a/fast3r_amd/csrc/f3r_attn.hip b/fast3r_amd/csrc/f3r_attn.hip
--- a/fast3r_amd/csrc/f3r_attn.hip
+++ b/fast3r_amd/csrc/f3r_attn.hip
@@ -386,6 +386,28 @@
   return p.family == ATTN_ASM ? f3r_attn_asm_name(*args, p) : hip[p.family];
 }
 
+extern "C" int f3r_attn_fwd_o8(const f3r_attn_args* args, uint32_t o8_off, f3r_stream_t stream) {
+  if (o8_off == 0) return f3r_attn_fwd(args, stream);
+  F3R_REQUIRE(args != nullptr, "f3r_attn_fwd_o8: null args");
+  const f3r_attn_args& a = *args;
+  int rc = attn_validate(a);
+  if (rc != F3R_OK) return rc;
+  auto unsupported = [](const char* what) { f3r_set_error("f3r_attn_fwd_o8: %s", what); return F3R_ERR_UNSUPPORTED; };
+  if (a.dtype != F3R_F16 || attn_head_dim(a) != 64 || a.qk_planes >= 2) return unsupported("the e4m3 copy of the output exists for fp16, head_dim 64, qk_planes 0 / 1");
+  if (a.state_out) return unsupported("a state_out launch parks its state and writes no output: there is nothing to copy");
+  const int64_t row8 = (int64_t)a.n_heads * 64;
+  if (o8_off % 4 != 0 || (int64_t)o8_off < 2 * row8 || (int64_t)o8_off + row8 > 2 * a.ldo)
+    return unsupported("o8_off must be a multiple of 4, at least n_heads * 128 and leave n_heads * 64 bytes inside the output row (2 * ldo bytes)");
+  if (a.tq == 0) return F3R_OK;
+  AttnPlan p;
+  rc = f3r_attn_plan(a, &p);
+  if (rc != F3R_OK) return rc;
+  if (p.family != ATTN_ASM)
+    return unsupported("only the hand-scheduled kernels write the e4m3 copy, and this launch does not go to them (kernel_sel 1, or not eligible: f3r_attn_args.kernel_sel)");
+  p.o8_off = o8_off;
+  return f3r_attn_asm_launch(a, p, (hipStream_t)stream);
+}
+
 extern "C" int f3r_attn_fwd(const f3r_attn_args* args, f3r_stream_t stream) {
   F3R_REQUIRE(args != nullptr, "f3r_attn_fwd: null args");
   const f3r_attn_args& a = *args;
diff --git a/fast3r_amd/csrc/f3r_attn_asm.hip b/fast3r_amd/csrc/f3r_attn_asm.hip
--- a/fast3r_amd/csrc/f3r_attn_asm.hip
+++ b/fast3r_amd/csrc/f3r_attn_asm.hip
@@ -26,13 +26,13 @@
   float* st_ml;
   uint64_t k_bs, vt_bs;
   uint32_t st_o_ld_b, st_ml_ld_b;
-  uint32_t tq, pad;
+  uint32_t tq, o8_off;
   f3r_attn_asm_seg seg[8];
   uint32_t* dbg;
   uint32_t* sched;
   uint32_t n_work, nx, nxy, nx_magic, nxy_magic, grid;
 };
-static_assert(sizeof(f3r_attn_asm_args) == 344 && offsetof(f3r_attn_asm_args, seg) == 112 && offsetof(f3r_attn_asm_args, dbg) == 304 &&
+static_assert(sizeof(f3r_attn_asm_args) == 344 && offsetof(f3r_attn_asm_args, o8_off) == 108 && offsetof(f3r_attn_asm_args, seg) == 112 && offsetof(f3r_attn_asm_args, dbg) == 304 &&
               offsetof(f3r_attn_asm_args, sched) == 312 && offsetof(f3r_attn_asm_args, n_work) == 320,
               "must match ARG_SIZE / ARG_SEG / ARG_DBG / ARG_SCHED of attn_gen.py");
 
@@ -44,14 +44,18 @@
 }
 AttnItem native_item(int hd, int planes) { return (hd == 64 && planes < 2) ? ATTN_ITEM_512 : ATTN_ITEM_256; }
 
-F3rCodeObject<12> g_kernels = {f3r_attn_asm_hsaco,
+F3rCodeObject<15> g_kernels = {f3r_attn_asm_hsaco,
                                {"f3r_attn_asm_f16", "f3r_attn_asm_bf16", "f3r_attn_asm_d80_f16", "f3r_attn_asm_d80_bf16", "f3r_attn_asm_d128_f16", "f3r_attn_asm_d128_bf16",
                                 "f3r_attn_asm_qk3_f16", "f3r_attn_asm_qk3f8_f16", "f3r_attn_asm_q256_f16", "f3r_attn_asm_q256_bf16", "f3r_attn_asm_f16_grp",
-                                "f3r_attn_asm_bf16_grp"}};
-
-hipFunction_t get_fn(int dtype, int hi, int planes, AttnItem item, bool grouped = false) {
+                                "f3r_attn_asm_bf16_grp", "f3r_attn_asm_f16_o8", "f3r_attn_asm_q256_f16_o8", "f3r_attn_asm_f16_grp_o8"}};
+
+hipFunction_t get_fn(int dtype, int hi, int planes, AttnItem item, bool grouped = false, bool o8 = false) {
   if (dtype < 0 || dtype > 1 || hi < 0) return nullptr;
   const bool hd64 = kHd[hi] == 64;
+  if (o8) {
+    if (!hd64 || dtype != F3R_F16 || planes >= 2) return nullptr;
+    return g_kernels.get(item != ATTN_ITEM_512 ? 13 : (grouped ? 14 : 12));
+  }
   if (planes >= 2) return (hd64 && dtype == F3R_F16) ? g_kernels.get(4 + planes) : nullptr;
   if (item != native_item(kHd[hi], planes)) return hd64 ? g_kernels.get(8 + dtype) : nullptr;
   if (grouped) return hd64 ? g_kernels.get(10 + dtype) : nullptr;
@@ -180,7 +184,7 @@
   const int hd = kHd[p.hd_index];
   const int wave_rows = attn_item_wave_rows(l.item);
   F3R_REQUIRE(l.rows >= wave_rows, "f3r_attn_fwd: a hand-scheduled launch of %lld query rows, fewer than the %d of one wave", (long long)l.rows, wave_rows);
-  hipFunction_t fn = get_fn(a.dtype, p.hd_index, p.planes, l.item, l.grouped);
+  hipFunction_t fn = get_fn(a.dtype, p.hd_index, p.planes, l.item, l.grouped, p.o8_off != 0);
   if (!fn) {
     f3r_set_error("f3r_attn_fwd: the embedded hand-scheduled kernel could not be loaded on this device");
     return F3R_ERR_LAUNCH;
@@ -203,6 +207,7 @@
   k.st_o_ld_b = (uint32_t)a.n_heads * (uint32_t)hd * 4u;
   k.st_ml_ld_b = (uint32_t)a.n_heads * 16u;
   k.tq = (uint32_t)l.rows;
+  k.o8_off = p.o8_off;
   k.dbg = a.dbg_counters;
   for (int s = 0; s < a.n_seg; ++s) {
     if (a.seg_len[s] == 0) continue;
diff --git a/fast3r_amd/csrc/f3r_dispatch.h b/fast3r_amd/csrc/f3r_dispatch.h
--- a/fast3r_amd/csrc/f3r_dispatch.h
+++ b/fast3r_amd/csrc/f3r_dispatch.h
@@ -130,6 +130,7 @@
   int hd_index = 0;
   int planes = 1;
   AttnAsmLaunch main, tail;
+  uint32_t o8_off = 0;
 };
 int f3r_attn_plan(const f3r_attn_args& a, AttnPlan* plan);
 bool f3r_attn_asm_plan(const f3r_attn_args& a, int64_t min_keys, AttnPlan* plan, const char** why);
diff --git a/fast3r_amd/csrc/f3r_gemm_asm.hip b/fast3r_amd/csrc/f3r_gemm_asm.hip
--- a/fast3r_amd/csrc/f3r_gemm_asm.hip
+++ b/fast3r_amd/csrc/f3r_gemm_asm.hip
@@ -33,12 +33,14 @@
 enum { ACT_SCALE = 3, ACT_ROPE = 4, FLAG_BIAS_ON_M = 1, FLAG_SKEW = 2 };
 
 enum { ROLE_F32 = 0, ROLE_LP = 1 };
-F3rCodeObject<6> g_kernels = {f3r_gemm_asm_hsaco, {"f3r_gemm_asm_f32_f16", "f3r_gemm_asm_f32_bf16", "f3r_gemm_asm_lp_f16", "f3r_gemm_asm_lp_bf16", "f3r_gemm_asm_f328_f16", "f3r_gemm_asm_lp8_f16"}};
+F3rCodeObject<7> g_kernels = {f3r_gemm_asm_hsaco, {"f3r_gemm_asm_f32_f16", "f3r_gemm_asm_f32_bf16", "f3r_gemm_asm_lp_f16", "f3r_gemm_asm_lp_bf16", "f3r_gemm_asm_f328_f16", "f3r_gemm_asm_lp8_f16",
+                                                   "f3r_gemm_asm_lp8a_f16"}};
 
 hipFunction_t get_fn(int role, int dtype, bool f8 = false) {
   if (dtype < 0 || dtype > 1 || (f8 && dtype != F3R_F16)) return nullptr;
   return g_kernels.get(f8 ? 4 + role : 2 * role + dtype);
 }
+hipFunction_t get_fn_scale_on_a() { return g_kernels.get(6); }
 
 int role_of(const f3r_gemm_args& a) { return a.out_f32 ? ROLE_F32 : ROLE_LP; }
 
@@ -205,7 +207,11 @@
   if ((int64_t)256 * a.lda * 2 >= (1ll << 32) || (int64_t)256 * a.Kpad * 3 >= (1ll << 32) || (int64_t)256 * a.ldvt * 2 >= (1ll << 32)) { *why = "row strides too large"; return false; }
   if ((a.M / 256) * (int64_t)(a.N / 256) >= (1ll << 24)) { *why = "grid too large"; return false; }
   if (!tile_map_exact(a.M / 256, 2 * (Dq / 256), Dq / 256) || !tile_map_exact(Dq / 256, a.M / 256, a.seq_len / 256)) { *why = "tile map: position x period reaches 2^32"; return false; }
-  if (get_fn(ROLE_LP, a.dtype) == nullptr || (f8 && get_fn(ROLE_LP, a.dtype, true) == nullptr)) { *why = "the embedded code object could not be loaded on this device"; return false; }
+  if (a.w_aux_f8 && !f8) { *why = "w_aux_f8 without F3R_SPLIT_W2F8"; return false; }
+  if (get_fn(ROLE_LP, a.dtype) == nullptr || (f8 && get_fn(ROLE_LP, a.dtype, true) == nullptr) || (a.w_aux_f8 && get_fn_scale_on_a() == nullptr)) {
+    *why = "the embedded code object could not be loaded on this device";
+    return false;
+  }
   return true;
 }
 
@@ -239,6 +245,26 @@
   if (rc != F3R_OK) return rc;
   f3r_gemm_asm_args v;
   memset(&v, 0, sizeof(v));
+  if (f8 && a.w_aux_f8) {
+    hipFunction_t fn_v = get_fn_scale_on_a();
+    if (!fn_v) return not_loaded();
+    v.A = a.W_aux;
+    v.W = a.A;
+    v.bias = a.bias ? a.bias + 2 * D : nullptr;
+    v.out = a.vt;
+    v.lda_b = (uint32_t)((int64_t)a.K * 3);
+    v.ldw_b = (uint32_t)(a.lda * 2);
+    v.ldo_b = (uint32_t)(a.ldvt * 2);
+    v.nk8 = (uint32_t)(a.K / 128);
+    v.nk = (uint32_t)(a.K / 64) + v.nk8;
+    v.nk1 = v.nk1_w = v.nk;
+    v.w_scale = a.w_scale + 2 * D;
+    v.scale = 1.0f;
+    v.flags = FLAG_BIAS_ON_M;
+    v.seg_stride = (int64_t)D * a.ldvt * 2;
+    v.tps = (uint32_t)(a.seq_len / 256);
+    return launch_tiles(fn_v, v, D, a.M, stream, skew, ROLE_LP);
+  }
   const int64_t kp_v = f8 ? (int64_t)2 * a.K : a.Kpad;
   v.A = f8 ? a.W_aux : (const void*)((const char*)a.W + (int64_t)2 * D * a.Kpad * 2);
   v.W = a.A;
diff --git a/fast3r_amd/fast3r.py b/fast3r_amd/fast3r.py
--- a/fast3r_amd/fast3r.py
+++ b/fast3r_amd/fast3r.py
@@ -51,6 +51,11 @@
           and _fills_chip(T, pb.qk_w8.shape[0]))
     fc1 = pb.fc1_w8 is not None and T % 256 == 0 and not pb.swiglu_hidden and _fills_chip(T, pb.fc1_w8.shape[0])
     return qk, fc1, fc1 and _fills_chip(T, pb.fc2_w8.shape[0])
+
+
+def _f8_proj(pb, T, seq_len):
+    return (pb.proj_w8 is not None and T % 256 == 0 and _fills_chip(T, pb.proj_w8.shape[0]) and pb.head_dim == 64 and not pb.causal
+            and pb.kv_group >= 1 and pb.kv_group & (pb.kv_group - 1) == 0 and seq_len % 64 == 0 and seq_len >= ops.ATTN_ASM_MIN_KEYS)
 
 
 class _GraphCache:
@@ -435,7 +440,7 @@
 
     def _block_ws(self, fmt, pb, T, D, n_seq, seq_len, dev, external_kv=False):
         hidden = pb.fc1_w.shape[0]
-        f8_rows = any(_f8_gemms(pb, T, seq_len))
+        f8_rows = any(_f8_gemms(pb, T, seq_len)) or (not external_kv and _f8_proj(pb, T, seq_len))
         return ops.BlockWorkspace(T, D, hidden, n_seq, seq_len, fmt.lp, dev, kv_dim=0 if external_kv else pb.kv_dim, f8_rows=f8_rows)
 
     def _block(self, fmt, x, pb, n_heads, scale, seq_len, n_seq, rope, kv_exchange=None, ws=None, kv_tap=None):
@@ -455,7 +460,7 @@
         f8_qkv, f8_fc1, f8_fc2 = _f8_gemms(pb, T, seq_len)
         if f8_qkv:
             rows1 = ops.layernorm_f8(x, pb.n1w, pb.n1b, pb.eps, out_rows=ws.rows8(D), rms=pb.rms)
-            ops.gemm_qkv(rows1, pb.qk_w8, pb.qkv_b, q, k, vt, seq_len, rope, q_scale=scale * ops.LOG2E, split="w2f8", w_scale=pb.qk_ws, w_aux=pb.v_w2)
+            ops.gemm_qkv(rows1, pb.qk_w8, pb.qkv_b, q, k, vt, seq_len, rope, q_scale=scale * ops.LOG2E, split="w2f8", w_scale=pb.qk_ws, w_aux=pb.v_w8)
             h = ws.h
         else:
             h, _ = ops.layernorm(x, pb.n1w, pb.n1b, pb.eps, lp, out_lp=ws.h, rms=pb.rms)
@@ -463,11 +468,14 @@
         if kv_tap is not None and kv_exchange is None:
             kv_tap(k, vt)
         o = h
+        f8_proj = kv_exchange is None and lp == torch.float16 and _f8_proj(pb, T, seq_len)
         gqa = dict(kv_group=pb.kv_group, causal=pb.causal, head_dim=pb.head_dim)
         if kv_exchange is None:
             Dkv = k.shape[1]
+            if f8_proj:
+                o = ws.rows8(D)
             ops.attention(q, o, n_heads, scale, [(k, vt, seq_len, seq_len * Dkv, Dkv * ldvt)], tq=seq_len, batch=n_seq,
-                          q_batch_stride=seq_len * D, o_batch_stride=seq_len * D, q_prescaled=True, **gqa)
+                          q_batch_stride=seq_len * D, o_batch_stride=seq_len * o.stride(0), q_prescaled=True, o8_off=2 * D if f8_proj else 0, **gqa)
         else:
             sharding = self.sharding
             sharding.begin_layer(kv_exchange)
@@ -495,7 +503,10 @@
                 kv_exchange.finish()
                 ops.attention(q, o, n_heads, scale, [kv_exchange.local_segment()], tq=seq_len, q_prescaled=True, **gqa)
             sharding.end_layer(kv_exchange)
-        ops.gemm(o, pb.proj_w, bias=pb.proj_b, res_f32=x, out_f32=x, split=sp)
+        if f8_proj:
+            ops.gemm(o, pb.proj_w8, bias=pb.proj_b, res_f32=x, out_f32=x, split="w2f8", w_scale=pb.proj_ws)
+        else:
+            ops.gemm(o, pb.proj_w, bias=pb.proj_b, res_f32=x, out_f32=x, split=sp)
         if f8_fc1:
             rows = ops.layernorm_f8(x, pb.n2w, pb.n2b, pb.eps, out_rows=ws.rows8(D), rms=pb.rms)
             if f8_fc2:
diff --git a/fast3r_amd/ops.py b/fast3r_amd/ops.py
--- a/fast3r_amd/ops.py
+++ b/fast3r_amd/ops.py
@@ -339,6 +339,7 @@
 
 
 LOG2E = 1.4426950408889634
+ATTN_ASM_MIN_KEYS = 2048
 
 
 def gemm_qkv(a, w, bias, q, k, vt, seq_len, rope=None, q_scale=0.0, rope_mode=0, split=None, a_lo=None, kernel_sel=0, q_dim=0, w_scale=None, w_aux=None):
@@ -351,12 +352,14 @@
         assert w_scale is not None and w_aux is not None and lp == torch.float16 and w_aux.dtype == lp
         K = Kpad = 2 * w.shape[1] // 3
         N = w.shape[0] + w_aux.shape[0]
-        assert w_aux.shape[1] == 2 * K and a.shape[1] * 2 >= 3 * K and w_scale.numel() == w.shape[0]
+        aux_f8 = w_aux.shape[1] * 2 == 3 * K
+        assert (aux_f8 or w_aux.shape[1] == 2 * K) and a.shape[1] * 2 >= 3 * K and w_scale.dtype == torch.int32 and w_scale.is_contiguous()
+        assert w_scale.numel() == (N if aux_f8 else w.shape[0])
     g = GemmArgs()
     g.A, g.W, g.bias = ptr(a), ptr(w), ptr(bias)
     g.M, g.N, g.K, g.Kpad, g.lda = M, N, K, Kpad, a.stride(0)
     if split == "w2f8":
-        g.w_scale, g.W_aux = ptr(w_scale), ptr(w_aux)
+        g.w_scale, g.W_aux, g.w_aux_f8 = ptr(w_scale), ptr(w_aux), int(aux_f8)
     g.a_mode, g.epi, g.act = F3R_A_PLAIN, F3R_EPI_QKV, F3R_ACT_NONE
     g.q, g.k, g.vt = ptr(q), ptr(k), ptr(vt)
     g.seq_len, g.ldvt = seq_len, vt.stride(-2)
@@ -488,7 +491,7 @@
 
 def attention(q, out, n_heads, scale, segments, tq=None, batch=1, q_batch_stride=0, o_batch_stride=0, q_prescaled=False,
               state=None, state_in=False, state_out=False, kv_group=1, causal=False, q_pos0=0, seg_pos0=None, kernel_sel=0, head_dim=64, qk_planes=1,
-              reserve_cus=0):
+              reserve_cus=0, o8_off=0):
     require_gpu(q, "q")
     lp = q.dtype
     assert 1 <= len(segments) <= F3R_MAX_SEG
@@ -534,7 +537,10 @@
         e0, e1 = torch.cuda.Event(enable_timing=True), torch.cuda.Event(enable_timing=True)
         e0.record()
     with _timed(4.0 * a.tq * sum(int(s_[2]) for s_ in segments) * head_dim * n_heads * batch, 0.0, "attention"):
-        check(_lib.lib().f3r_attn_fwd(ctypes.byref(a), stream_ptr()), "f3r_attn_fwd")
+        if o8_off:
+            check(_lib.entry("f3r_attn_fwd_o8")(ctypes.byref(a), int(o8_off), stream_ptr()), "f3r_attn_fwd_o8")
+        else:
+            check(_lib.lib().f3r_attn_fwd(ctypes.byref(a), stream_ptr()), "f3r_attn_fwd")
     if ATTN_TIMER is not None:
         e1.record()
         t_k = sum(int(s[2]) for s in segments)
diff --git a/fast3r_amd/packing.py b/fast3r_amd/packing.py
--- a/fast3r_amd/packing.py
+++ b/fast3r_amd/packing.py
@@ -8,12 +8,13 @@
     __slots__ = ("n1w", "n1b", "n2w", "n2b", "eps", "qkv_w", "qkv_b", "proj_w", "proj_b", "fc1_w", "fc1_b", "fc2_w", "fc2_b",
                  "rms", "rope_mode", "swiglu_hidden", "q_dim", "kv_dim", "kv_group", "causal", "head_dim", "fc1_split",
                  "fc1_w8", "fc1_ws", "fc2_w8", "fc2_ws",
-                 "qk_w8", "qk_ws", "v_w2")
+                 "qk_w8", "qk_ws", "v_w8",
+                 "proj_w8", "proj_ws")
 
     def __init__(self, norm1, norm2):
         self.n1w, self.n1b, self.n2w, self.n2b = (_f32(getattr(n, a, None)) for n in (norm1, norm2) for a in ("weight", "bias"))
         self.eps = norm1.eps
-        self.fc1_w8 = self.fc1_ws = self.fc2_w8 = self.fc2_ws = self.qk_w8 = self.qk_ws = self.v_w2 = None
+        self.fc1_w8 = self.fc1_ws = self.fc2_w8 = self.fc2_ws = self.qk_w8 = self.qk_ws = self.v_w8 = self.proj_w8 = self.proj_ws = None
         self.rms, self.rope_mode, self.swiglu_hidden = False, 0, 0
         self.fc1_split = None
         self.head_dim = 64
@@ -41,8 +42,12 @@
     wq = blk.attn.qkv.weight.detach().float()
     Dm = wq.shape[0] // 3
     if fmt.low_f8 and wq.shape[1] % 128 == 0 and Dm % 256 == 0 and head_dim == 64:
-        p.qk_w8, p.qk_ws = ops.pack_linear_weight_f8(wq[:2 * Dm])
-        p.v_w2 = ops.pack_linear_weight(wq[2 * Dm:], lp, True)
+        p.qk_w8, qk_ws = ops.pack_linear_weight_f8(wq[:2 * Dm])
+        p.v_w8, v_ws = ops.pack_linear_weight_f8(wq[2 * Dm:])
+        p.qk_ws = torch.cat([qk_ws, v_ws]).contiguous()
+    wp = blk.attn.proj.weight.detach().float()
+    if fmt.low_f8 and wp.shape[1] % 128 == 0 and wp.shape[0] % 256 == 0 and head_dim == 64:
+        p.proj_w8, p.proj_ws = ops.pack_linear_weight_f8(wp)
     return p
 
 
diff --git a/include/f3r.h b/include/f3r.h
--- a/include/f3r.h
+++ b/include/f3r.h
@@ -97,7 +97,7 @@
   float* fin_conf;
   int32_t fin_n_out, fin_depth_mode, fin_conf_mode;
   float fin_vmin, fin_vmax;
-  int32_t reserved0;
+  int32_t w_aux_f8;
 } f3r_gemm_args;
 
 typedef enum { F3R_SPLIT_NONE = 0, F3R_SPLIT_W2 = 1, F3R_SPLIT_X3 = 2, F3R_SPLIT_W2F8 = 3, F3R_SPLIT_X3F8 = 4 } f3r_split;
@@ -146,6 +146,7 @@
 
 int f3r_attn_fwd(const f3r_attn_args* args, f3r_stream_t stream);
 const char* f3r_attn_kernel_name(const f3r_attn_args* args);
+int f3r_attn_fwd_o8(const f3r_attn_args* args, uint32_t o8_off, f3r_stream_t stream);
 
 int f3r_upsample2x(const void* in, const void* in_lo, void* out, void* out_lo, int batch, int h, int w, int C, int out_h, int out_w,
                    int dtype, f3r_stream_t stream);
```
